# chto/linna

Hardware: AMD Instinct MI355X
Metric: emulator log-likelihood evals/sec (higher is better)
Workload: dtype f32; 1 GPU; 33-D Gaussian, 4x512 MLP emulator (33->512x4->33), nwalkers=4096 batched log-likelihood per GPU (BASELINE configs[1]); nwalkers_per_gpu=4096, launch=direct launches, parallelism=walkers sharded, 1 rank(s), no data-path collective

## Files before the change

### include/linna_hip.h

```cpp
#ifndef LINNA_HIP_H
#define LINNA_HIP_H
#include <stddef.h>
#include <stdint.h>

#ifdef __cplusplus
extern "C" {
#endif

#define LINNA_ABI_VERSION 12

typedef struct linna_ctx linna_ctx_t;
typedef struct linna_net linna_net_t;
typedef struct linna_logprob linna_logprob_t;
typedef struct linna_graph linna_graph_t;

int linna_abi_version(void);
const char* linna_last_error(void);
#define LINNA_OK 0
#define LINNA_ERR_INVALID (-1)
#define LINNA_ERR_HIP (-2)
#define LINNA_ERR_UNSUPPORTED (-3)
#define LINNA_ERR_INTERNAL (-4)
int linna_debug_raise(int kind);
int linna_ctx_create(int device, linna_ctx_t** out);
// ... 61 lines not shown
                     const float* W, int ldw, float* dX, int lddx, const float* Xmask, int ldxm,
                     float* dW, int lddw, float* db, int B, int K, int N, float scale, void* stream);

#define LINNA_LD(k) (((k) + 3) & ~3)
#define LINNA_OP_LINEAR 0
#define LINNA_OP_RESBLOCK 1
#define LINNA_OP_INSKIP 2

typedef struct {
    uint32_t struct_size;
    int op;
    int K, C, N;
    int relu;
    float alpha;
    const float *W, *b;
    const float *W1, *b1, *W2, *b2, *Ws;
    float *gW, *gb, *gW1, *gb1, *gW2, *gb2, *gWs;
} linna_layer_t;

typedef struct {
    const float* cscale; const float* cshift;
    int cexp; const float* cpost; const float* cshift2;
} linna_colmap_t;

int linna_net_create(linna_ctx_t* ctx, const linna_layer_t* layers, int nlayers, int in_size,
                     linna_net_t** out);
int linna_net_destroy(linna_net_t* net);
int linna_net_prepare(linna_net_t* net, int backward, int input_grad);
size_t linna_net_fwd_ws_bytes(const linna_net_t* net, int B);
size_t linna_net_bwd_ws_bytes(const linna_net_t* net, int B);
int linna_net_forward(linna_net_t* net, const float* X, int ldx, int B, void* ws, float* OUT, int ldo,
                      const linna_colmap_t* outmap, void* stream);
int linna_net_backward(linna_net_t* net, const float* X, int ldx, int B, void* fwd_ws, void* bwd_ws,
                       const float* dOUT, int lddo, float* dX, int lddx, int param_grads, void* stream);
int linna_net_train_launches(const linna_net_t* net, int B);
int linna_net_set_train_precision(linna_net_t* net, int precision);
int linna_net_train_precision(const linna_net_t* net, int* out);
int linna_net_stream_state(const linna_net_t* net, int* fwd, int* dx, int* dx_input);

int linna_prior_map_fwd(linna_ctx_t* ctx, const float* Z, int ldz, int B, int nin, const int* is_flat,
                        const float* a1, const float* a2, const int* log10_flag, const float* xmean,
                        const float* xstd, float* X, int ldx, float* THETA, int ldt, void* stream);
int linna_prior_map_bwd(linna_ctx_t* ctx, const float* Z, int ldz, int B, int nin, const int* is_flat,
                        const float* a1, const float* a2, const int* log10_flag, const float* xstd,
                        const float* dX, int lddx, float* dZ, int lddz, void* stream);

int linna_gauss_loglike_diag(linna_ctx_t* ctx, const float* D, int ldd, int B, int nout, const float* w,
                             const float* Z, int ldz, int nin, float temperature, float* out,
                             void* stream);
int linna_gauss_loglike_dense(linna_ctx_t* ctx, const float* D, int ldd, int B, int nout,
                              const float* S, int lds, const float* Z, int ldz, int nin,
                              float temperature, float* scratch, float* out, void* stream);

typedef struct {
    uint32_t struct_size;
    int nin, nout;
    const int* is_flat; const float* a1; const float* a2;
    const int* log10_flag; const float* xmean; const float* xstd;
    linna_colmap_t outmap;
    const float* S; int lds;
    const float* Ssym;
    const float* w;
    const float* gscale;
    float temperature;
    const float* Sfac;
} linna_logprob_desc_t;

int linna_logprob_create(linna_ctx_t* ctx, linna_net_t* net, const linna_logprob_desc_t* desc,
                         linna_logprob_t** out);
int linna_logprob_destroy(linna_logprob_t* lp);
int linna_weights_changed(linna_ctx_t* ctx);
#define LINNA_PRECISION_FP32 0
#define LINNA_PRECISION_BF16 1
int linna_logprob_set_precision(linna_logprob_t* lp, int precision);
int linna_logprob_precision(const linna_logprob_t* lp, int* out);
int linna_logprob_set_grad_precision(linna_logprob_t* lp, int precision);
int linna_logprob_grad_precision(const linna_logprob_t* lp, int* out);
int linna_logprob_set_dense_grad(linna_logprob_t* lp, int on);
int linna_logprob_dense_grad(const linna_logprob_t* lp, int* out);
int linna_engine_rows(int rows);
int linna_dense_tri(int mode);
int linna_serve_plain(int on);
int linna_serve_plain_sched(int hand);
int linna_program_plain(const linna_layer_t* layers, int nlayers, int in_size, int rows, int dense_nout);
int linna_logprob_serve_plain(linna_logprob_t* lp, int B, int* out);
int linna_logprob_grad_launches(linna_logprob_t* lp, int B, int* out);
int linna_slice_fusion(int mask);
int linna_program_describe(const linna_layer_t* layers, int nlayers, int in_size, int rows, int dense_nout, char* buf,
                           size_t n);
int linna_program_describe_grad_bf16(const linna_layer_t* layers, int nlayers, int in_size, int rows, char* buf, size_t n);
int linna_program_describe_grad_dense(const linna_layer_t* layers, int nlayers, int in_size, int nout, int tri, int rows,
                                      char* buf, size_t n);
size_t linna_logprob_ws_bytes(const linna_logprob_t* lp, int B, int with_grad);
int linna_logprob_eval(linna_logprob_t* lp, const float* Z, int ldz, int B, void* ws, float* lnP,
                       float* THETA, int ldt, void* stream);
int linna_logprob_eval_if(linna_logprob_t* lp, const float* Z, int ldz, int B, void* ws, float* lnP,
                          float* THETA, int ldt, const int* gate, void* stream);
int linna_logprob_eval_slice_points(linna_logprob_t* lp, const float* coords, int ldc, int ndim, const int* S_idx,
                                    int ns, const float* DIR, int ldd, const float* w, int nrep, float* lnP,
                                    const int* gate, void* stream);
int linna_logprob_grad(linna_logprob_t* lp, const float* Z, int ldz, int B, void* ws, float* lnP,
                       float* G, int ldg, void* stream);
int linna_logprob_grad_leapfrog(linna_logprob_t* lp, float* Q, int ldq, int B, void* ws, float* lnP, float* G, int ldg,
                                float* P, int ldp, const float* mass, float eps_kick, float eps_drift, void* stream);

typedef struct {
    uint32_t struct_size;
    int nout;
    const float* sigma; const float* ymean; const float* ystd;
    const float* data_norm;
    const float* Cinv; int ldc;
    int ylog;
} linna_loss_desc_t;

size_t linna_loss_scratch_bytes(int B, int nout);
int linna_chi2_md(linna_ctx_t* ctx, const linna_loss_desc_t* d, const float* Y, int ldy, int nrows,
                  float* scratch, float* den, void* stream);
int linna_chi2_ratio_loss_fwd_bwd(linna_ctx_t* ctx, const linna_loss_desc_t* d, const float* PRED,
                                  int ldp, const float* Y, int ldy, const float* den, const int* ROWS,
                                  int B, float* scratch, float* loss_rows, float* loss_mean,
                                  float* dPRED, int lddp, float inv_batch, void* stream);
int linna_net_prepare_loss(linna_net_t* net, const linna_loss_desc_t* d);
int linna_loss_targets(linna_ctx_t* ctx, const linna_loss_desc_t* d, const float* Y, int ldy, int nrows, float* YN, int ldyn,
                       void* stream);
int linna_net_forward_loss(linna_net_t* net, const linna_loss_desc_t* d, const float* X, int ldx, const int* ROWS, int B,
                           const int* log10_flag, const float* xmean, const float* xstd, float* XB, int ldxb, void* ws,
                           float* PRED, int ldp, const float* YN, int ldyn, const float* den, float inv_batch,
                           float* loss_rows, float* loss_mean, float* dPRED, int lddp,
                           float* hyper, int* step_dev, float beta1, float beta2, void* stream);
int linna_net_train_step(linna_net_t* net, const linna_loss_desc_t* d, const float* X, int ldx, const int* ROWS, int B,
                         const int* log10_flag, const float* xmean, const float* xstd, float* XB, int ldxb, void* fwd_ws,
                         float* PRED, int ldp, const float* YN, int ldyn, const float* den, float inv_batch,
                         float* loss_rows, float* loss_mean, float* dPRED, int lddp, void* bwd_ws,
                         float* hyper, int* step_dev, float beta1, float beta2, void* stream);
int linna_val_rows(linna_ctx_t* ctx, const linna_loss_desc_t* d, const float* PRED, int ldp,
                   const float* Y, int ldy, const float* den, int B, float* scratch, float* loss_rows,
                   float* frac_rows, void* stream);
int linna_val_metrics(linna_ctx_t* ctx, const float* loss_rows, const float* frac_rows, int n, const float* last_train_loss,
                      float* out, void* stream);
int linna_gather_xform(linna_ctx_t* ctx, const float* X, int ldx, const int* ROWS, int B, int nin,
                       const int* log10_flag, const float* xmean, const float* xstd, float* XB, int ldxb,
                       void* stream);
int linna_adamw_step(linna_ctx_t* ctx, float* p, const float* g, float* m, float* v, size_t n,
                     float* hyper, int* step_dev, float beta1, float beta2, float eps,
                     int prepared ,
                     void* stream);
int linna_net_adamw_step(linna_net_t* net, int B, float* p, const float* g, float* m, float* v, size_t n,
                         float* hyper, int* step_dev, float beta1, float beta2, float eps, int prepared, void* stream);
int linna_net_train_step_update(linna_net_t* net, const linna_loss_desc_t* d, const float* X, int ldx, const int* ROWS, int B,
                                const int* log10_flag, const float* xmean, const float* xstd, float* XB, int ldxb,
                                void* fwd_ws, float* PRED, int ldp, const float* YN, int ldyn, const float* den,
                                float inv_batch, float* loss_rows, float* loss_mean, float* dPRED, int lddp, void* bwd_ws,
                                float* params, float* m, float* v, size_t n, float* hyper, int* step_dev, float beta1,
                                float beta2, float eps, void* stream);

int linna_stretch_propose(linna_ctx_t* ctx, const float* coords, int ldc, int ndim, const int* S_idx,
                          int ns, const float* ccoords, int ldcc, const int* C_idx, int nc, uint64_t seed,
                          const int* step_dev, int stream_id, float a, float* Q, int ldq, float* factors,
                          void* stream);
int linna_stretch_accept(linna_ctx_t* ctx, float* coords, int ldc, int ndim, float* logp,
                         const int* S_idx, int ns, const float* Q, int ldq, const float* logp_new,
                         const float* factors, uint64_t seed, const int* step_dev, int stream_id,
                         int* naccept, void* stream);
int linna_stretch_half_step(linna_logprob_t* lp, float* coords, int ldc, int ndim, float* logp,
                            const int* S_idx, int ns, const float* ccoords, int ldcc, const int* C_idx,
                            int nc, uint64_t seed, const int* step_dev, int step_offset, int stream_id,
// ... 132 lines not shown
```

### linna_amd/_lib.py

```python
import ctypes as C
import os

import torch

_HERE = os.path.dirname(os.path.abspath(__file__))
LIB_PATH = os.environ.get("LINNA_LIB_PATH") or os.path.join(_HERE, "liblinna_hip.so")
ABI_VERSION = 12
RHAT_BLOCK = 128

c_float_p = C.c_void_p
c_int_p = C.c_void_p


class _Sized(C.Structure):

    def __init__(self, *a, **k):
        C.Structure.__init__(self, *a, **k)
        self.struct_size = C.sizeof(type(self))


def sized_array(cls, n):
    arr = (cls * n)()
    for i in range(n):
        arr[i].struct_size = C.sizeof(cls)
# ... 27 lines not shown
    _fields_ = [("cscale", C.c_void_p), ("cshift", C.c_void_p), ("cexp", C.c_int), ("cpost", C.c_void_p),
                ("cshift2", C.c_void_p)]


class LogprobDesc(_Sized):
    _fields_ = [("struct_size", C.c_uint32), ("nin", C.c_int), ("nout", C.c_int), ("is_flat", C.c_void_p), ("a1", C.c_void_p), ("a2", C.c_void_p),
                ("log10_flag", C.c_void_p), ("xmean", C.c_void_p), ("xstd", C.c_void_p), ("outmap", ColMap),
                ("S", C.c_void_p), ("lds", C.c_int), ("Ssym", C.c_void_p), ("w", C.c_void_p), ("gscale", C.c_void_p),
                ("temperature", C.c_float), ("Sfac", C.c_void_p)]


class HmcState(_Sized):
    _fields_ = [("struct_size", C.c_uint32), ("B", C.c_int), ("ld", C.c_int), ("seed", C.c_uint64), ("step_dev", C.c_void_p),
                ("mass", C.c_void_p), ("X", C.c_void_p), ("lnp", C.c_void_p), ("G", C.c_void_p), ("P", C.c_void_p),
                ("Q", C.c_void_p), ("lnp_new", C.c_void_p), ("Gnew", C.c_void_p), ("H0", C.c_void_p)]


class LossDesc(_Sized):
    _fields_ = [("struct_size", C.c_uint32), ("nout", C.c_int), ("sigma", C.c_void_p), ("ymean", C.c_void_p), ("ystd", C.c_void_p),
                ("data_norm", C.c_void_p), ("Cinv", C.c_void_p), ("ldc", C.c_int), ("ylog", C.c_int)]


OP_LINEAR, OP_RESBLOCK, OP_INSKIP = 0, 1, 2
COMM_ID_BYTES = 128
LAY_K, LAY_MN = 0, 1
CHEES_HEAD, CHEES_LR, CHEES_BETA1, CHEES_BETA2, CHEES_ADAM_EPS, CHEES_ALPHA_FLOOR, CHEES_MAX_STEPS = 12, 0.025, 0.9, 0.999, 1e-8, 1e-3, 64

_V, _I, _F, _SZ, _U64 = C.c_void_p, C.c_int, C.c_float, C.c_size_t, C.c_uint64
_I64, _D = C.c_int64, C.c_double
_PV = C.POINTER(C.c_void_p)

_SIGNATURES = {
    "linna_abi_version": (_I, []),
    "linna_last_error": (C.c_char_p, []),
    "linna_debug_raise": (_I, [_I]),
    "linna_ctx_create": (_I, [_I, _PV]),
    "linna_ctx_destroy": (_I, [_V]),
    "linna_stream_sync": (_I, [_V]),
    "linna_graph_begin": (_I, [_V]),
    "linna_graph_end": (_I, [_V, _PV]),
    "linna_graph_launch": (_I, [_V, _V]),
    "linna_graph_destroy": (_I, [_V]),
    "linna_event_create": (_I, [_PV]),
    "linna_event_record": (_I, [_V, _V]),
    "linna_event_elapsed_ms": (_I, [_V, _V, C.POINTER(C.c_float)]),
    "linna_event_destroy": (_I, [_V]),
    "linna_comm_unique_id": (_I, [_V]),
    "linna_comm_init": (_I, [_V, _I, _I, _V]),
    "linna_comm_destroy": (_I, [_V]),
    "linna_comm_info": (_I, [_V, C.POINTER(C.c_int), C.POINTER(C.c_int), C.POINTER(C.c_int)]),
    "linna_allreduce_sum_f32": (_I, [_V, _V, _SZ, _V]),
    "linna_allgather_f32": (_I, [_V, _V, _V, _SZ, _V]),
    "linna_broadcast_f32": (_I, [_V, _V, _SZ, _I, _V]),
    "linna_gemm_f32": (_I, [_V, C.POINTER(Gemm), _V]),
    "linna_gemm_dot_slots": (_I, [_I, _I]),
    "linna_linear_fwd": (_I, [_V, _V, _I, _V, _I, _V, _V, _I, _I, _I, _I, _I, _F, _V, _I, _V]),
    "linna_resblock_fwd": (_I, [_V, _V, _I, _V, _V, _V, _V, _V, _V, _I, _V, _I, _I, _I, _I, _I, _V]),
    "linna_linear_bwd": (_I, [_V, _V, _I, _V, _I, _V, _I, _V, _I, _V, _I, _V, _I, _V, _I, _I, _I, _F, _V]),
    "linna_net_create": (_I, [_V, C.POINTER(Layer), _I, _I, _PV]),
    "linna_net_destroy": (_I, [_V]),
    "linna_net_prepare": (_I, [_V, _I, _I]),
    "linna_net_fwd_ws_bytes": (_SZ, [_V, _I]),
    "linna_net_bwd_ws_bytes": (_SZ, [_V, _I]),
    "linna_net_forward": (_I, [_V, _V, _I, _I, _V, _V, _I, C.POINTER(ColMap), _V]),
    "linna_net_backward": (_I, [_V, _V, _I, _I, _V, _V, _V, _I, _V, _I, _I, _V]),
    "linna_net_stream_state": (_I, [_V, _V, _V, _V]),
    "linna_prior_map_fwd": (_I, [_V, _V, _I, _I, _I, _V, _V, _V, _V, _V, _V, _V, _I, _V, _I, _V]),
    "linna_prior_map_bwd": (_I, [_V, _V, _I, _I, _I, _V, _V, _V, _V, _V, _V, _I, _V, _I, _V]),
    "linna_gauss_loglike_diag": (_I, [_V, _V, _I, _I, _I, _V, _V, _I, _I, _F, _V, _V]),
    "linna_gauss_loglike_dense": (_I, [_V, _V, _I, _I, _I, _V, _I, _V, _I, _I, _F, _V, _V, _V]),
    "linna_logprob_create": (_I, [_V, _V, C.POINTER(LogprobDesc), _PV]),
    "linna_logprob_destroy": (_I, [_V]),
    "linna_weights_changed": (_I, [_V]),
    "linna_logprob_set_precision": (_I, [_V, _I]),
    "linna_logprob_precision": (_I, [_V, _V]),
    "linna_logprob_set_grad_precision": (_I, [_V, _I]),
    "linna_logprob_grad_precision": (_I, [_V, _V]),
    "linna_logprob_set_dense_grad": (_I, [_V, _I]),
    "linna_logprob_dense_grad": (_I, [_V, _V]),
    "linna_engine_rows": (_I, [_I]),
    "linna_dense_tri": (_I, [_I]),
    "linna_serve_plain": (_I, [_I]),
    "linna_serve_plain_sched": (_I, [_I]),
    "linna_program_plain": (_I, [_V, _I, _I, _I, _I]),
    "linna_logprob_serve_plain": (_I, [_V, _I, _V]),
    "linna_logprob_grad_launches": (_I, [_V, _I, _V]),
    "linna_slice_fusion": (_I, [_I]),
    "linna_net_train_launches": (_I, [_V, _I]),
    "linna_net_set_train_precision": (_I, [_V, _I]),
    "linna_net_train_precision": (_I, [_V, _V]),
    "linna_program_describe": (_I, [_V, _I, _I, _I, _I, _V, C.c_size_t]),
    "linna_program_describe_grad_bf16": (_I, [_V, _I, _I, _I, _V, C.c_size_t]),
    "linna_program_describe_grad_dense": (_I, [_V, _I, _I, _I, _I, _I, _V, C.c_size_t]),
    "linna_logprob_ws_bytes": (_SZ, [_V, _I, _I]),
    "linna_logprob_eval": (_I, [_V, _V, _I, _I, _V, _V, _V, _I, _V]),
    "linna_logprob_grad": (_I, [_V, _V, _I, _I, _V, _V, _V, _I, _V]),
    "linna_logprob_grad_leapfrog": (_I, [_V, _V, _I, _I, _V, _V, _V, _I, _V, _I, _V, _F, _F, _V]),
    "linna_loss_scratch_bytes": (_SZ, [_I, _I]),
    "linna_chi2_md": (_I, [_V, C.POINTER(LossDesc), _V, _I, _I, _V, _V, _V]),
    "linna_chi2_ratio_loss_fwd_bwd": (_I, [_V, C.POINTER(LossDesc), _V, _I, _V, _I, _V, _V, _I, _V, _V, _V, _V, _I, _F, _V]),
    "linna_net_prepare_loss": (_I, [_V, C.POINTER(LossDesc)]),
    "linna_loss_targets": (_I, [_V, C.POINTER(LossDesc), _V, _I, _I, _V, _I, _V]),
    "linna_net_forward_loss": (_I, [_V, C.POINTER(LossDesc), _V, _I, _V, _I, _V, _V, _V, _V, _I, _V, _V, _I, _V, _I, _V, _F, _V, _V, _V, _I,
                                    _V, _V, _F, _F, _V]),
    "linna_net_train_step": (_I, [_V, C.POINTER(LossDesc), _V, _I, _V, _I, _V, _V, _V, _V, _I, _V, _V, _I, _V, _I, _V, _F, _V, _V, _V, _I,
                                  _V, _V, _V, _F, _F, _V]),
    "linna_net_train_step_update": (_I, [_V, C.POINTER(LossDesc), _V, _I, _V, _I, _V, _V, _V, _V, _I, _V, _V, _I, _V, _I, _V, _F, _V, _V, _V, _I,
                                         _V, _V, _V, _V, _SZ, _V, _V, _F, _F, _F, _V]),
    "linna_val_rows": (_I, [_V, C.POINTER(LossDesc), _V, _I, _V, _I, _V, _I, _V, _V, _V, _V]),
    "linna_val_metrics": (_I, [_V, _V, _V, _I, _V, _V, _V]),
    "linna_gather_xform": (_I, [_V, _V, _I, _V, _I, _I, _V, _V, _V, _V, _I, _V]),
    "linna_adamw_step": (_I, [_V, _V, _V, _V, _V, _SZ, _V, _V, _F, _F, _F, _I, _V]),
    "linna_net_adamw_step": (_I, [_V, _I, _V, _V, _V, _V, _SZ, _V, _V, _F, _F, _F, _I, _V]),
    "linna_stretch_propose": (_I, [_V, _V, _I, _I, _V, _I, _V, _I, _V, _I, _U64, _V, _I, _F, _V, _I, _V, _V]),
    "linna_stretch_accept": (_I, [_V, _V, _I, _I, _V, _V, _I, _V, _I, _V, _V, _U64, _V, _I, _V, _V]),
    "linna_logprob_eval_if": (_I, [_V, _V, _I, _I, _V, _V, _V, _I, _V, _V]),
    "linna_logprob_eval_slice_points": (_I, [_V, _V, _I, _I, _V, _I, _V, _I, _V, _I, _V, _V, _V]),
    "linna_stretch_half_step": (_I, [_V, _V, _I, _I, _V, _V, _I, _V, _I, _V, _I, _U64, _V, _I, _I, _F, _V, _V]),
    "linna_stretch_run": (_I, [_V, _V, _I, _I, _V, _I, _V, _I, _I, _U64, _V, _I, _F, _V, _V, _V, _V]),
    "linna_chain_append_t": (_I, [_V, _V, _I, _I, _I, _I, _I, _V, _I, _I64, _V]),
    "linna_acorr_update": (_I, [_V, _V, _I, _I, _I, _I64, _I64, _I64, _I64, _I, _I, _V, _V, _I, _V]),
    "linna_acorr_scratch_bytes": (_SZ, [_I, _I, _I]),
    "linna_acorr_tau": (_I, [_V, _V, _I, _I, _I, _I, _I64, _I64, _I, _V, _V, _D, _V, _V, _V]),
    "linna_chain_meanstd": (_I, [_V, _V, _I, _I, _I, _I64, _I64, _I64, _V, _V]),
    "linna_chain_block_moments": (_I, [_V, _V, _I, _I, _I64, _I64, _V, _V]),
    "linna_chain_rhat": (_I, [_V, _V, _I, _I, _I, _I64, _I64, _V, _I64, _V, _V]),
    "linna_acorr_ess_scratch_bytes": (_SZ, [_I, _I, _I]),
    "linna_acorr_ess": (_I, [_V, _V, _I, _I, _I, _I, _I64, _I64, _I, _V, _V, _V, _V, _V]),
    "linna_chain_rank_rhat_scratch_bytes": (_SZ, [_I, _I, _I64, _I]),
    "linna_chain_rank_rhat": (_I, [_V, _V, _I, _I, _I, _I64, _I64, _V, _SZ, _V, _V, _V]),
    "linna_hmc_init": (_I, [_V, _I, _I, _V, _U64, _V, _V, _V, _I, _V, _I, _V, _V]),
    "linna_hmc_start": (_I, [_V, _I, _I, _V, _U64, _V, _V, _V, _I, _V, _I, _F, _F, _V, _I, _V, _I, _V, _I, _V, _V]),
    "linna_hmc_kick_drift": (_I, [_V, _I, _I, _V, _F, _F, _V, _I, _V, _I, _V, _I, _V]),
    "linna_hmc_accept": (_I, [_V, _I, _I, _V, _U64, _V, _V, _V, _I, _V, _I, _V, _V, _I, _V, _V, _I, _V, _V, _V, _V]),
    "linna_hmc_start_eps": (_I, [_V, _I, _I, _V, _U64, _V, _I, _V, _V, _I, _V, _I, _V, _F, _F, _V, _I, _V, _I, _V, _I, _V, _V]),
    "linna_hmc_kick_drift_eps": (_I, [_V, _I, _I, _V, _V, _F, _F, _V, _I, _V, _I, _V, _I, _V]),
    "linna_logprob_grad_leapfrog_eps": (_I, [_V, _V, _I, _I, _V, _V, _V, _I, _V, _I, _V, _V, _F, _F, _V]),
    "linna_hmc_accept_adapt": (_I, [_V, _I, _I, _V, _U64, _V, _I, _V, _V, _I, _V, _I, _V, _V, _I, _V, _V, _I, _V, _V, _V, _V,
                                    _V, _V, _V, _V, _V, _I, _F, _V, _V, _V]),
    "linna_hmc_run": (_I, [_V, _V, _V, _V, _V, _V, _V, _V, _I, _F, _I, _I, _I, _V, _V, _V, _V, _V]),
    "linna_hmc_find_epsilon": (_I, [_V, _V, _V, _V, _V, _V, _V, _I, _I, _V]),
    "linna_hmc_moments": (_I, [_V, _I, _I, _V, _I, _V, _V]),
    "linna_hmc_mass_from_moments": (_I, [_V, _I, _V, _V, _I, _V]),
    "linna_hmc_run_moments": (_I, [_V, _V, _V, _V, _V, _V, _V, _V, _I, _F, _I, _I, _I, _V, _V, _V, _V, _V, _V]),
    "linna_hmc_comoments_doubles": (_SZ, [_I]),
    "linna_hmc_comoments": (_I, [_V, _I, _I, _V, _I, _V, _V]),
    "linna_hmc_chol_from_comoments": (_I, [_V, _I, _V, _V, _I, _V, _I, _V]),
    "linna_hmc_kick_drift_dense": (_I, [_V, _I, _I, _V, _I, _V, _F, _F, _V, _I, _V, _I, _V, _I, _V, _I, _V]),
    "linna_hmc_run_dense": (_I, [_V, _V, _V, _V, _I, _V, _V, _V, _V, _V, _I, _F, _I, _I, _I, _V, _V, _V, _V, _V, _V]),
    "linna_hmc_find_epsilon_dense": (_I, [_V, _V, _V, _V, _I, _V, _V, _V, _V, _I, _I, _V]),
    "linna_hmc_chees_doubles": (_SZ, [_I]),
    "linna_hmc_chees_begin": (_I, [_V, _I, _I, _V, _I, _V, _V, _V]),
    "linna_hmc_chees_end": (_I, [_V, _I, _I, _V, _V, _I, _V, _I, _V, _I, _V, _V, _V, _V, _I, _D, _I, _V]),
    "linna_step_increment": (_I, [_V, _V, _V]),
    "linna_slice_init": (_I, [_V, _V, _V, _I, _V, _I, _V, _I, _I, _V, _U64, _V, _I, _V, _I, _V, _V, _V, _V, _I, _V]),
    "linna_slice_points": (_I, [_V, _V, _I, _I, _V, _I, _V, _I, _V, _V, _I, _I, _V]),
    "linna_slice_expand": (_I, [_V, _V, _V, _V, _V, _V, _V, _I, _V, _I, _V]),
    "linna_slice_draw": (_I, [_V, _V, _V, _V, _V, _V, _I, _U64, _V, _I, _I, _I, _V]),
    "linna_slice_shrink": (_I, [_V, _V, _V, _V, _V, _V, _V, _V, _V, _I, _V, _I, _I, _V]),
    "linna_slice_commit": (_I, [_V, _V, _I, _I, _V, _V, _I, _V, _I, _V, _V, _V]),
    "linna_slice_half_step": (_I, [_V, _V, _I, _I, _V, _V, _I, _V, _I, _V, _I, _V, _U64, _V, _I, _V, _I, _V, _I, _V, _I, _V, _V, _V, _V, _V, _V, _V, _I, _I, _V, _I, _V]),
}
EXPORTED = tuple(_SIGNATURES)

_lib = None

# ... 65 lines not shown
        raise LinnaHipError("expected dtype %s, got %s" % (dtype, t.dtype))
    if not t.is_contiguous():
        raise LinnaHipError("expected a contiguous tensor")
    return C.c_void_p(t.data_ptr())


def iptr(t):
    return ptr(t, torch.int32)


def ld4(w):
    return (int(w) + 3) & ~3


class _Stage(object):
    __slots__ = ("name", "t0")

    def __init__(self, name):
        self.name = name

    def __enter__(self):
        if stage_profile.current is not None:
            import time
            self.t0 = time.perf_counter()
        return self

    def __exit__(self, *exc):
        d = stage_profile.current
        if d is not None:
            import time
            d[self.name] = d.get(self.name, 0.0) + time.perf_counter() - self.t0
        return False


def stage(name):
    return _Stage(name)


class stage_profile(object):
    current = None

    def __init__(self, d):
        self.d = d

    def __enter__(self):
        self.prev, stage_profile.current = stage_profile.current, self.d
        return self.d

    def __exit__(self, *exc):
        stage_profile.current = self.prev
        return False


class quiet_gc(object):

    def __enter__(self):
        import gc
        self.on = gc.isenabled() and os.environ.get("LINNA_QUIET_GC", "1") != "0"
        if self.on:
            gc.freeze()
        return self

    def __exit__(self, *exc):
        import gc
        if self.on:
            gc.unfreeze()
        return False


def slice_fusion(mask=-1):
    prev = load().linna_slice_fusion(int(mask))
    if prev < 0:
        check(prev)
    return prev


def serve_plain_sched(hand=-1):
    prev = load().linna_serve_plain_sched(int(hand))
    if prev < 0:
        check(prev)
    return prev


def serve_plain(on=-1):
    prev = load().linna_serve_plain(int(on))
    if prev < 0:
        check(prev)
    return prev


def engine_rows(rows=0):
    prev = load().linna_engine_rows(int(rows))
    if prev < 0:
        check(prev)
    return prev
```

### linna_amd/csrc/api.hip

```cpp
#include "common.h"

#include <stdarg.h>
#include <stdio.h>
#include <string.h>
#include <cstring>
#include <string>
#include <vector>
#include <atomic>
#include <new>
#include <stdlib.h>

namespace linna {

static thread_local std::string g_err;

void set_error(const char* fmt, ...) {
    char buf[512];
    va_list ap;
    va_start(ap, fmt);
    vsnprintf(buf, sizeof buf, fmt, ap);
    va_end(ap);
    g_err = buf;
}

// ... 1053 lines not shown
    if (lp->d.outmap.cexp) { set_error("logprob_set_grad_precision: no bf16 gradient: the ypositive (exp) output map has no gradient path"); return LINNA_ERR_UNSUPPORTED; }
    if (!lp->d.w || !lp->d.gscale) { set_error("logprob_set_grad_precision: no bf16 gradient: it needs a diagonal likelihood with gscale"); return LINNA_ERR_UNSUPPORTED; }
    const NsPlan g = net_stream_plan(NS_GRAD_INPUT_BF16, n->Lfull.data(), (int)n->Lfull.size(), n->in_size);
    if (!g.ok) {
        set_error("logprob_set_grad_precision: no bf16 gradient for this network: %s", g.why ? g.why : "not eligible");
        return LINNA_ERR_UNSUPPORTED;
    }
    if (!lp->packed_gbf.ready() && lp->packed_gbf.alloc(g.packed_floats) != LINNA_OK) {
        set_error("logprob_set_grad_precision: hipMalloc(bf16 gradient weight stream) failed");
        return LINNA_ERR_HIP;
    }
    lp->grad_precision = precision;
    return LINNA_OK;
} LINNA_CATCH_INT
int linna_logprob_grad_precision(const linna_logprob_t* lp, int* out) try {
    if (!lp || !out) { set_error("logprob_grad_precision: null argument"); return LINNA_ERR_INVALID; }
    *out = lp->grad_precision;
    return LINNA_OK;
} LINNA_CATCH_INT
int linna_logprob_set_dense_grad(linna_logprob_t* lp, int on) try {
    if (!lp) { set_error("logprob_set_dense_grad: null handle"); return LINNA_ERR_INVALID; }
    if (on != 0 && on != 1) { set_error("logprob_set_dense_grad: %d (0 layered, 1 one launch)", on); return LINNA_ERR_INVALID; }
    if (!on) { lp->dense_grad = false; return LINNA_OK; }
    const linna_net* n = lp->net;
    const linna_logprob_desc_t& d = lp->d;
    if (lp->bf16()) { set_error("logprob_set_dense_grad: a bf16 handle has no dense-covariance gradient (fp32 only)"); return LINNA_ERR_UNSUPPORTED; }
    if (d.w) { set_error("logprob_set_dense_grad: the covariance is diagonal: its gradient is one launch already where the network has the program"); return LINNA_ERR_UNSUPPORTED; }
    if (d.outmap.cexp) { set_error("logprob_set_dense_grad: the ypositive (exp) output map has no gradient path"); return LINNA_ERR_UNSUPPORTED; }
    if (!d.Sfac) {
        set_error("logprob_set_dense_grad: no factored inverse covariance (Sfac): it is not positive definite, or LINNA_DENSE_FACTORED=0");
        return LINNA_ERR_UNSUPPORTED;
    }
    if (n->has_inskip) { set_error("logprob_set_dense_grad: an input-skip network has no one-launch gradient"); return LINNA_ERR_UNSUPPORTED; }
    const NsDense dn = lp->dense();
    const NsPlan g = net_stream_plan(NS_GRAD_INPUT_DENSE, n->L.data(), (int)n->L.size(), n->in_size, &dn);
    if (!g.ok) {
        set_error("logprob_set_dense_grad: no one-launch dense gradient for this network: %s", g.why ? g.why : "not eligible");
        return LINNA_ERR_UNSUPPORTED;
    }
    if (!lp->packed_gd.ready() && lp->packed_gd.alloc(g.packed_floats) != LINNA_OK) {
        set_error("logprob_set_dense_grad: hipMalloc(dense gradient weight stream) failed");
        return LINNA_ERR_HIP;
    }
    for (int e = 0; e < 3; ++e) lp->gd_fits[e] = net_stream_grad_dense_fits(n->L.data(), (int)n->L.size(), n->in_size, &dn, 16 >> e);
    lp->dense_grad = true;
    return LINNA_OK;
} LINNA_CATCH_INT
int linna_logprob_dense_grad(const linna_logprob_t* lp, int* out) try {
    if (!lp || !out) { set_error("logprob_dense_grad: null argument"); return LINNA_ERR_INVALID; }
    *out = lp->dense_grad ? 1 : 0;
    return LINNA_OK;
} LINNA_CATCH_INT
int linna_program_describe_grad_dense(const linna_layer_t* layers, int nlayers, int in_size, int nout, int tri, int rows, char* buf, size_t n) try {
    if (!layers || nlayers < 1 || !buf || !n || nout < 1 || tri < 0 || tri > 2) { set_error("program_describe_grad_dense: bad arguments"); return LINNA_ERR_INVALID; }
    TRY(check_layers(layers, nlayers, "program_describe_grad_dense"));
    if (layers[nlayers - 1].N != nout) { set_error("program_describe_grad_dense: %d columns for a network of %d outputs", nout, layers[nlayers - 1].N); return LINNA_ERR_INVALID; }
    static float dummy[2];
    const NsDense dn{dummy, (nout + 3) & ~3, dummy + 1, dummy + 1, 1, tri};
    return net_stream_describe(NS_GRAD_INPUT_DENSE, layers, nlayers, in_size, &dn, rows, buf, n);
} LINNA_CATCH_INT
int linna_program_describe_grad_bf16(const linna_layer_t* layers, int nlayers, int in_size, int rows, char* buf, size_t n) try {
    if (!layers || nlayers < 1 || !buf || !n) { set_error("program_describe_grad_bf16: bad arguments"); return LINNA_ERR_INVALID; }
    TRY(check_layers(layers, nlayers, "program_describe_grad_bf16"));
    return net_stream_describe(NS_GRAD_INPUT_BF16, layers, nlayers, in_size, nullptr, rows, buf, n);
} LINNA_CATCH_INT
int linna_program_describe(const linna_layer_t* layers, int nlayers, int in_size, int rows, int dense_nout, char* buf, size_t n) try {
    if (!layers || nlayers < 1 || !buf || !n) { set_error("program_describe: bad arguments"); return LINNA_ERR_INVALID; }
    TRY(check_layers(layers, nlayers, "program_describe"));
    static float dummy;
    if (dense_nout == -1) return net_stream_describe(ns_grad_kind(layers, nlayers), layers, nlayers, in_size, nullptr, rows, buf, n);
    const int dn_cols = dense_nout < -1 ? -dense_nout : dense_nout;
    NsDense dn{&dummy, (dn_cols + 3) & ~3, nullptr, nullptr, dense_nout < -1 ? 1 : 0, net_stream_dense_tri(-1)};
    if (dn_cols > 0) return net_stream_describe(NS_SERVE_DENSE, layers, nlayers, in_size, &dn, rows, buf, n);
    return net_stream_describe(NS_SERVE, layers, nlayers, in_size, nullptr, rows, buf, n);
} LINNA_CATCH_INT
int linna_serve_plain(int on) try {
    if (on < -1 || on > 1) { set_error("linna_serve_plain: %d (-1 query, 0 or 1)", on); return LINNA_ERR_INVALID; }
    return net_stream_serve_plain(on);
} LINNA_CATCH_INT
int linna_serve_plain_sched(int hand) try {
    if (hand < -1 || hand > 1) { set_error("linna_serve_plain_sched: %d (-1 query, 0 or 1)", hand); return LINNA_ERR_INVALID; }
    return net_stream_serve_plain_sched(hand);
} LINNA_CATCH_INT
int linna_program_plain(const linna_layer_t* layers, int nlayers, int in_size, int rows, int dense_nout) try {
    if (!layers || nlayers < 1) { set_error("program_plain: bad arguments"); return LINNA_ERR_INVALID; }
    TRY(check_layers(layers, nlayers, "program_plain"));
    if (dense_nout != 0) return 0;
    return net_stream_program_plain(NS_SERVE, layers, nlayers, in_size, nullptr, rows) ? 1 : 0;
} LINNA_CATCH_INT
int linna_logprob_serve_plain(linna_logprob_t* lp, int B, int* out) try {
    if (!lp || !out || B < 1) { set_error("logprob_serve_plain: bad arguments"); return LINNA_ERR_INVALID; }
    static float lnP;
    *out = lp_eval_route(lp, false).route == LP_EVAL_ONE &&
           net_stream_takes_plain(lp->kind(), net_layers(lp->net, lp->kind()), lp_output(lp), NsRun{nullptr, 0, B, &lnP}, nullptr, nullptr,
                                  net_stream_rows(B), nullptr);
    return LINNA_OK;
} LINNA_CATCH_INT
int linna_dense_tri(int mode) try {
    if (mode < -1 || mode > 2) { set_error("linna_dense_tri: %d (-1 query, 0, 1 or 2)", mode); return LINNA_ERR_INVALID; }
    return net_stream_dense_tri(mode);
} LINNA_CATCH_INT
static std::atomic<int> g_slice_fusion{7};
static bool slice_derive_enabled() { return (g_slice_fusion.load() & 1) != 0; }
int linna_slice_fusion(int mode) try {
    if (mode < -1 || mode > 7) { set_error("linna_slice_fusion: %d (-1 query, or a mask of bits 0-2)", mode); return LINNA_ERR_INVALID; }
    return mode < 0 ? g_slice_fusion.load() : g_slice_fusion.exchange(mode);
} LINNA_CATCH_INT
int linna_engine_rows(int rows) try {
    const int prev = net_stream_force_rows(rows);
    if (prev < 0) { set_error("linna_engine_rows: %d (0, 4, 8 or 16)", rows); return LINNA_ERR_INVALID; }
    if (prev != rows) g_weights_epoch.fetch_add(1);
    return prev;
} LINNA_CATCH_INT
size_t linna_logprob_ws_bytes(const linna_logprob_t* lp, int B, int with_grad) try {
    return (lp_layout(lp, B, with_grad).total + 16) * sizeof(float);
} LINNA_CATCH_SIZE

int linna_logprob_eval(linna_logprob_t* lp, const float* Z, int ldz, int B, void* ws, float* lnP, float* TH, int ldt,
                       void* stream) try {
    if (!lp || !Z || !ws || !lnP || B < 1) { set_error("logprob_eval: bad arguments"); return LINNA_ERR_INVALID; }
    return lp_forward(lp, NsRun{Z, ldz, B, lnP, nullptr, TH, ldt}, static_cast<float*>(ws), lp_layout(lp, B, 0), stream, false);
} LINNA_CATCH_INT

int linna_logprob_eval_if(linna_logprob_t* lp, const float* Z, int ldz, int B, void* ws, float* lnP, float* TH, int ldt,
                          const int* gate, void* stream) try {
    if (!lp || !Z || !ws || !lnP || B < 1) { set_error("logprob_eval_if: bad arguments"); return LINNA_ERR_INVALID; }
    return lp_forward(lp, NsRun{Z, ldz, B, lnP, gate, TH, ldt}, static_cast<float*>(ws), lp_layout(lp, B, 0), stream, false);
} LINNA_CATCH_INT

struct SliceDerive { const float* Z0; const float* L; const float* R; const float* Ze; int m, nt; uint64_t seed; const int* step_dev; int stream_id; const int* flags; };
struct SlicePoints { const float* coords; int ldc, ndim; const int* S_idx; int ns; const float* DIR; int ldd; };
static int lp_eval_slice_points(linna_logprob_t* lp, const SlicePoints& pt, const float* w, int nrep, float* lnP, const int* gate,
                                const int* list, const int* count, int mul, int b_engine, void* stream, const SliceDerive* sd = nullptr,
                                const SliceBegin* sb = nullptr) {
    if (!lp || !pt.coords || !pt.S_idx || !pt.DIR || !w || !lnP || pt.ns < 1 || nrep < 1) {
        set_error("logprob_eval_slice_points: bad arguments"); return LINNA_ERR_INVALID;
    }
    if (pt.ndim != lp->d.nin) { set_error("logprob_eval_slice_points: ndim %d, log-probability has %d parameters", pt.ndim, lp->d.nin); return LINNA_ERR_INVALID; }
    if (!lp_runs_fused_move(lp)) {
        set_error("logprob_eval_slice_points: this log-probability does not run the whole-network kernel");
        return LINNA_ERR_UNSUPPORTED;
    }
    const float* packed = nullptr; int rows = 16;
    TRY(lp_refresh_stream(lp, b_engine > 0 ? b_engine : nrep * pt.ns, stream, &packed, &rows));
    NsMove mv{const_cast<float*>(pt.coords), pt.ldc, nullptr, pt.S_idx, w, 0, list, pt.ns, 0ull, count, mul, 0, 0.f, nullptr, 1};
    mv.sb = sb;
    if (sd) {
        mv.sl_Z0 = sd->Z0; mv.sl_L = sd->L; mv.sl_R = sd->R; mv.sl_Zt = sd->Ze; mv.sl_m = sd->m; mv.sl_nt = sd->nt;
        mv.sl_seed = sd->seed; mv.sl_step = sd->step_dev; mv.sl_stream = sd->stream_id; mv.sl_flags = sd->flags;
    }
    return lp_launch(lp, packed, rows, NsRun{pt.DIR, pt.ldd, nrep * pt.ns, lnP, gate}, &mv, nullptr, stream);
}
int linna_logprob_eval_slice_points(linna_logprob_t* lp, const float* coords, int ldc, int ndim, const int* S_idx, int ns,
                                    const float* DIR, int ldd, const float* w, int nrep, float* lnP, const int* gate,
                                    void* stream) try {
    return lp_eval_slice_points(lp, SlicePoints{coords, ldc, ndim, S_idx, ns, DIR, ldd}, w, nrep, lnP, gate, nullptr, nullptr, 0, 0, stream);
} LINNA_CATCH_INT

int linna_slice_half_step(linna_logprob_t* lp, float* coords, int ldc, int ndim, float* logp, const int* S_idx, int ns,
                          const float* ccoords, int ldcc, const int* C_idx, int nc, const float* mu, uint64_t seed,
                          int* step_dev, int half, const int* m_sched, int nexp_rounds, const int* nt_sched, int nshr_rounds,
                          float* DIR, int ldd, float* state, int* flags, float* W, float* Wd, float* Zt, int* list, int* counters,
                          int zero_totals, int bump_step, const int* expect_rows, int maxsteps, void* stream) try {
    if (!lp || !coords || !logp || !S_idx || !ccoords || !C_idx || !mu || !step_dev || !DIR || !state || !flags || !W || !Wd ||
        !Zt || !list || !counters || ns < 1 || nc < 2 || !m_sched || !nt_sched || nexp_rounds < 1 || nshr_rounds < 1 || (half != 0 && half != 1)) {
        set_error("slice_half_step: bad arguments"); return LINNA_ERR_INVALID;
// ... 697 lines not shown
```

### linna_amd/csrc/common.h

```cpp
#pragma once
#include <hip/hip_runtime.h>
#include <stdint.h>
#include <exception>
#include "../../include/linna_hip.h"


typedef float f32x4 __attribute__((ext_vector_type(4)));
typedef float f32x16 __attribute__((ext_vector_type(16)));

namespace linna {

struct U4 { uint32_t x, y, z, w; };
__device__ __forceinline__ U4 philox4x32_10(U4 c, uint32_t k0, uint32_t k1) {
#pragma unroll
    for (int r = 0; r < 10; ++r) {
        const uint64_t p0 = (uint64_t)0xD2511F53u * c.x;
        const uint64_t p1 = (uint64_t)0xCD9E8D57u * c.z;
        U4 n;
        n.x = (uint32_t)(p1 >> 32) ^ c.y ^ k0;
        n.y = (uint32_t)p1;
        n.z = (uint32_t)(p0 >> 32) ^ c.w ^ k1;
        n.w = (uint32_t)p0;
        c = n;
        k0 += 0x9E3779B9u; k1 += 0xBB67AE85u;
// ... 212 lines not shown
                        const float* xstd, float* XB, int ldxb, hipStream_t s);
int launch_colsum(const float* dZ, int ld, int B, int N, float scale, float* db, hipStream_t s);
int launch_adamw(float* p, const float* g, float* m, float* v, size_t n, float* hyper, int* step_dev, float b1, float b2,
                 float eps, hipStream_t s);
int launch_adamw_prepare(float* hyper, int* step_dev, float b1, float b2, hipStream_t s);
int launch_stretch_propose(const float* coords, int ldc, int ndim, const int* S, int ns, const float* ccoords, int ldcc,
                           const int* C, int nc, uint64_t seed, const int* step_dev, int stream_id, float a, float* Q,
                           int ldq, float* factors, hipStream_t s);
int launch_stretch_accept(float* coords, int ldc, int ndim, float* logp, const int* S, int ns, const float* Q, int ldq,
                          const float* lp_new, const float* factors, uint64_t seed, const int* step_dev, int stream_id,
                          int* naccept, hipStream_t s);
int launch_hmc_start(int B, int ndim, const float* mass, uint64_t seed, const int* step_dev, const float* lnp, const float* P0,
                     int ldp0, const float* G, int ldg, float ek, float ed, const float* X, int ldx, float* P, int ldp, float* Q,
                     int ldq, float* H0, hipStream_t s, const float* eps = nullptr, int step_off = 0);
int launch_hmc_kick_drift(int B, int ndim, const float* mass, float ek, float ed, const float* G, int ldg, float* P,
                          int ldp, float* Q, int ldq, hipStream_t s, const float* eps = nullptr);
struct HmcAdapt { float* eps; float* epsbar; float* Hbar; const float* mu; int* m; int Madapt; float delta; };
int launch_hmc_accept(int B, int ndim, const float* mass, uint64_t seed, const int* step_dev, int step_off, const float* H0,
                      const float* P, int ldp, const float* Qn, int ldq, const float* lnp_new, const float* Gn, int ldg,
                      const float* U, float* X, int ldx, float* lnp, float* G, int* naccept, float* alpha,
                      const HmcAdapt& ad, float* chain, float* logps, hipStream_t s);
int launch_hmc_find_eps_init(int B, int ndim, uint64_t seed, const int* step_dev, int step_off, float* R0, int ldr, float* eps,
                             int* state, hipStream_t s);
int launch_hmc_find_eps(int B, int ndim, const float* mass, const float* H0, const float* P, int ldp, const float* lnp_new,
                        const float* Gn, int ldg, float* eps, int* state, int* nactive, hipStream_t s);
int launch_hmc_moments(int B, int ndim, const float* X, int ldx, double* mom, hipStream_t s);
int launch_hmc_mass_from_moments(int ndim, double* mom, float* mass, int reset, hipStream_t s);
int launch_hmc_comoments(int B, int ndim, const float* X, int ldx, double* mom, hipStream_t s);
int launch_hmc_chol_from_comoments(int ndim, double* mom, float* Cm, int ldc, int* info, int reset, hipStream_t s);
int launch_hmc_kick_drift_dense(int B, int ndim, const float* Cm, int ldc, const float* eps, float ek, float ed, const float* G,
                                int ldg, float* W, int ldw, const float* X, int ldx, float* Q, int ldq, hipStream_t s);
int launch_hmc_chees_begin(int B, int ndim, const float* X, int ldx, double* state, double* r0, hipStream_t s);
int launch_hmc_chees_end(int B, int ndim, const float* mass, const float* Cm, int ldc, const float* Q, int ldq, const float* P, int ldp,
                         const float* alpha, const double* r0, double* state, float* eps, int M, double delta, int max_steps,
                         hipStream_t s);
int launch_slice_points(const float* coords, int ldc, int ndim, const int* S, int ns, const float* DIR, int ldd,
                        const float* w, float* Q, int ldq, int nrep, hipStream_t s);
int launch_slice_expand(const float* Z0, const float* ZL, const float* ZR, float* L, float* R, int* flags, int ns,
                        int* counters, int slot, hipStream_t s);
int launch_slice_draw(const float* L, const float* R, const int* S, float* W, const int* flags, int ns, uint64_t seed,
                      const int* step_dev, int stream_id, int round, int ntrial, hipStream_t s);
int launch_slice_shrink(const float* Z0, const float* Zt, float* L, float* R, const float* W, int* flags, float* Wacc,
                        float* Zacc, int ns, int* counters, int slot, int ntrial, hipStream_t s);
int launch_slice_begin(const SliceBegin& b, const int* S, int ns, int ndim, float* W, hipStream_t s);
int launch_slice_expand_multi(const float* Z0, const float* Zt, float* L, float* R, const int* S, int* flags, int ns, int m,
                              int m_next, int* counters, int slot, int prev_slot, float* W, float* Wd, int* list, uint64_t seed,
                              const int* step_dev, int stream_id_shrink, int ntrial, hipStream_t s);
int launch_slice_shrink_multi(const SliceRound& a, hipStream_t s);
int launch_slice_commit(float* coords, int ldc, int ndim, float* logp, const int* S, int ns, const float* DIR, int ldd,
                        const float* Wacc, const float* Zacc, hipStream_t s);
int launch_step_increment(int* step, hipStream_t s);

struct NsDense { const float* S; int lds; const float* cscale; const float* cshift; int factored = 0;
                 int tri = 2; };
int net_stream_dense_tri(int mode);
enum NsKind {
    NS_SERVE,
    NS_SERVE_DENSE,
    NS_SERVE_BF16,
    NS_STORE,
    NS_TRAIN_FWD,
    NS_DX,
    NS_DX_INPUT,
    NS_GRAD_INPUT,
    NS_TRAIN_STEP,
    NS_TRAIN_STEP_BF16,
    NS_GRAD_INPUT_BF16,
    NS_GRAD_INPUT_WIDE,
    NS_GRAD_INPUT_DENSE,
};
inline bool ns_kind_full_layers(NsKind k) { return k == NS_SERVE || k == NS_SERVE_DENSE || k == NS_SERVE_BF16; }
struct NsPlan { bool ok; size_t packed_floats; bool grad_ok; const char* why; };
NsPlan net_stream_plan(NsKind kind, const linna_layer_t* layers, int nl, int in_size, const NsDense* dn = nullptr);
int net_stream_rows(int B);
int net_stream_force_rows(int rows);
inline NsKind ns_grad_kind(const linna_layer_t* layers, int nl) { return nl >= 1 && layers[nl - 1].N > 64 ? NS_GRAD_INPUT_WIDE : NS_GRAD_INPUT; }
bool net_stream_grad_fits(const linna_layer_t* layers, int nl, int in_size, int rows);
bool net_stream_grad_dense_fits(const linna_layer_t* layers, int nl, int in_size, const NsDense* dn, int rows);
int launch_net_stream_pack(NsKind kind, const linna_layer_t* layers, int nl, int in_size, float* packed, int rows, const NsDense* dn,
                           hipStream_t s);
int net_stream_describe(NsKind kind, const linna_layer_t* layers, int nl, int in_size, const NsDense* dn, int rows, char* buf, size_t n);
int net_stream_serve_plain(int on);
int net_stream_serve_plain_sched(int hand);
bool net_stream_program_plain(NsKind kind, const linna_layer_t* layers, int nl, int in_size, const NsDense* dn, int rows);
bool net_stream_launch_plain_ok(bool cscale, bool cshift, bool w, bool cexp, bool lnP, bool D, bool TH, bool gate);
struct NsNet { const linna_layer_t* layers; int nl, in_size; };
struct NsInput { int nin; const int* is_flat; const float* a1; const float* a2; const int* lg; const float* xmean; const float* xstd; };
struct NsOutput { const float* cscale; const float* cshift; const float* cpost; const float* cshift2; const float* w; float T; };
struct NsRun { const float* Z; int ldz; int B; float* lnP; const int* gate = nullptr; float* TH = nullptr; int ldt = 0; float* D = nullptr; int ldd = 0; };
struct NsOpBufs { float* y; int ldy; float* t; int ldt; const float* x; int ldx; const float* gate; float* dprev; int ldp; float* dt; int lddt; };
struct NsPost { const float* rows; int n; float scale; float* out; int* step; float* hyper; float b1, b2; };
int launch_net_stream_dx(const NsNet& net, const float* packed, const float* dOUT, int lddo, int B, const NsOpBufs* ops, int with_input,
                         int rows, hipStream_t s, const NsPost* post = nullptr);
struct NsMove {
    float* coords; int ldc; float* logp; const int* S;
    const float* cc; int ldcc; const int* C; int nc;
    unsigned long long seed; const int* step; int step_off; int stream; float a; int* naccept;
    int slice;
    float* chain = nullptr; float* lps = nullptr;
    const float* sl_Z0 = nullptr; const float* sl_L = nullptr; const float* sl_R = nullptr; const float* sl_Zt = nullptr;
    int sl_m = 0, sl_nt = 0; unsigned long long sl_seed = 0; const int* sl_step = nullptr; int sl_stream = 0;
    const int* sl_flags = nullptr;
    const SliceBegin* sb = nullptr;
};
int launch_net_stream_store(const NsNet& net, const float* packed, const float* X, int ldx, int B, const NsOpBufs* ops,
                            const float* cscale, const float* cshift, int rows, hipStream_t s);
struct NsTrainLoss { const float* YN; int ldyn;
                     const float* den; float inv_batch; float* loss_rows; float* dP; int lddp; };
struct NsBatch { const float* X; int ldx; const int* ROWS; int B; const int* lg; const float* xmean; const float* xstd; float* XB; int ldxb; };
int launch_loss_targets(const float* Y, int ldy, int n, const linna_loss_desc_t& d, float* YN, int ldyn, hipStream_t s);
int launch_net_stream_train(const NsNet& net, const float* packed, const NsBatch& b, const NsOpBufs* ops, const NsTrainLoss& L,
                            const NsDense& dn, int rows, hipStream_t s);
int launch_net_stream_train_bwd(const NsNet& net, const float* packed, const NsBatch& b, const NsOpBufs* ops, const NsTrainLoss& L,
                                const NsDense& dn, int rows, hipStream_t s, const NsPost* post,
                                bool bf = false);
struct NsLeap { float* P; int ldp; float* Q; const float* mass; float ek, ed; const float* eps; };
struct NsGrad { const float* gscale; float* G; int ldg; NsLeap leap; };
constexpr int AS_MAXR = 26, AS_MAXW = 14, AS_MAXB = 12;
struct AsPlace { float* out; float scale; int trans, koff, ncols, type, ncg, steps, G, first0, first1; };
struct AsMat { int N, ld; AsPlace pl[2]; };
struct AsBias { float* out; float scale; int N; };
struct AsRange { unsigned off4, n4, blk0; short kind, idx; };
struct AsArgs { AsRange r[AS_MAXR]; AsMat w[AS_MAXW]; AsBias b[AS_MAXB]; int nr, small; unsigned nblocks; };
__device__ __forceinline__ size_t as_slot(const AsPlace& q, int small, int nn, int kk) {
    const int nl = nn & 63, ks = kk >> 4, kr = kk & 15;
    int w, g;
    if (q.type == 0) { w = (nn & 511) >> 6; g = ((nn >> 9) ? q.first1 : q.first0) + ks; }
    else { const int kp = ks / q.steps; w = kp * q.ncg + (nn >> 6); g = q.first0 + (ks - kp * q.steps); }
    const int t = small ? kr >> 2 : nl >> 4, lane = small ? nl : (nl & 15) + 16 * (kr >> 2);
    return ((((size_t)w * q.G + g) * 4 + t) * 64 + lane) * 4 + (kr & 3);
}
__device__ __forceinline__ size_t as_slot_bf16(const AsPlace& q, int nn, int kk) {
    const int nl = nn & 63, ks = kk >> 5, kr = kk & 31;
    int w, g;
    if (q.type == 0) { w = (nn & 511) >> 6; g = ((nn >> 9) ? q.first1 : q.first0) + ks; }
    else { const int kp = ks / q.steps; w = kp * q.ncg + (nn >> 6); g = q.first0 + (ks - kp * q.steps); }
    return ((((size_t)w * q.G + g) * 4 + (kr >> 3)) * 64 + nl) * 8 + (kr & 7);
}
typedef __bf16 bf16x4_t __attribute__((ext_vector_type(4)));
__device__ __forceinline__ void adamw_one(float& pi, float gi, float& mi, float& vi, float lr, float wd, float bc1, float sbc2,
                                          float beta1, float beta2, float eps) {
    pi = pi * (1.f - lr * wd);
    mi = mi + (gi - mi) * (1.f - beta1);
    vi = vi * beta2 + (1.f - beta2) * gi * gi;
    const float denom = sqrtf(vi) / sbc2 + eps;
    pi = pi - (lr / bc1) * (mi / denom);
}
int net_stream_adamw_args(const linna_layer_t* layers, int nl, int in_size, int rows, const float* params, size_t nflat,
                          float* s_fwd, const NsDense* dn, float* s_dx, AsArgs* out, int merged = 0);
int launch_adamw_streams(const AsArgs& a, float* p, const float* g, float* m, float* v, const float* hyper, float b1, float b2,
                         float eps, hipStream_t s, bool bf = false);
int launch_net_stream_grad2(const NsNet& net, const float* packed, const NsRun& r, const NsInput& in, const NsOutput& out, const NsGrad& gr,
                            int rows, hipStream_t s, bool bf = false);
int launch_net_stream_grad_dense(const NsNet& net, const float* packed, const NsRun& r, const NsInput& in, float T, const NsGrad& gr,
                                 int rows, const NsDense& dn, hipStream_t s);
bool net_stream_takes_plain(NsKind kind, const NsNet& net, const NsOutput& out, const NsRun& r, const NsMove* mv, const NsGrad* gr, int rows,
                            const NsDense* dn);
int launch_net_stream(NsKind kind, const NsNet& net, const float* packed, const NsRun& r, const NsInput& in, const NsOutput& out,
                      const NsMove* mv, const NsGrad* gr, int rows, const NsDense* dn, hipStream_t s);

int launch_chain_append_t(const float* block, int ldb, int nsteps, int nw, int ndim, int wstride, float* CT, int nwp,
                          int64_t row0, hipStream_t s);
int launch_acorr_update(const float* CT, int nd, int nwp, int nwc, int64_t a0, int64_t a1, int64_t lo, int64_t hi, int k0, int k1,
                        double* S, double* T, int remove, hipStream_t s);
size_t acorr_scratch_doubles(int nser, int kuse, int nd);
int launch_acorr_tau(const float* CT, int ndim, int nwp, int nwc, int nlive, int64_t lo, int64_t hi, int kuse, const double* S,
// ... 33 lines not shown
```

### linna_amd/csrc/net_program.h

```cpp
#pragma once
#include "common.h"
#include <memory>
#include <vector>

namespace linna {

constexpr int NS_ROWS = 16;
constexpr int NS_NW = 8;
constexpr int NS_NT = 4;
constexpr int NS_MAXSEG = 20;
constexpr int NS_SEGCAP = 22;
constexpr int NS_MAXRUN = 40;
constexpr unsigned NS_STEP_B = NS_NT * 1024;
constexpr int NS_LDS_BYTES = 160 * 1024;
constexpr int AS_BLOCK = 64;
enum { NS_WIDE = 0, NS_SPLIT = 1, NS_SIDE = 2 };

struct NsSeg {
    int type, steps, passes, bias_off;
    int dst_col, relu, kslice, zext;
    int ncg_log2;
    int mask_store, mask_apply;
    int x0_n;
    int x0_col;
    int kcl, side_off;
};

struct NsPackSeg {
    const float* Wa; int lda, Ka, Kapad;
    const float* Wb; int ldb, Kb; float alpha;
    const float* b; float bscale;
    const float* b2; float b2scale;
    int N, type, steps, passes, bias_off, bias_pad, ncg;
    int transA;
    int transB;
    const float* rscale; const float* rshift;
    int kc, side_off;
    int koff2;
    const float* kscale;
};

struct NsProgram {
    std::vector<NsPackSeg> pack;
    std::vector<NsSeg> seg;
    int G = 0, LD = 0, kpad0 = 0, nout = 0, bias_total = 0;
    int Gstride = 0, nseg_f = 0, mask_slots = 0;
    size_t packed_floats = 0;
    int dense = 0, u_col = 0, u_same = 0;
    int x0_keep = 0;
    size_t side_f4 = 0;
    bool bf = false;
    int f32seg = -1;
    bool ok = false, grad_ok = false;
    bool dxi_ok = false;
    bool train_ok = false;
    int nops = 0;
    std::vector<int> seg_op, seg_hidden;
    size_t lds_for(int rows, bool grad) const;
};

int ns_seg_steps(const NsSeg& s);
int ns_forced_rows_resolved();
typedef std::shared_ptr<const NsProgram> NsProgramRef;
NsProgramRef ns_program(NsKind kind, const linna_layer_t* layers, int nl, int in_size, const NsDense* dn, int rows);

bool ns_program_plain(const NsProgram& p);
int ns_seg_cols(const NsProgram& p, const linna_layer_t* layers, int i);
struct NsGates {
    int gbit[NS_SEGCAP], mbit[NS_SEGCAP];
    int ncols = 0;
    bool ok = true;
    size_t lds0 = 0, lds = 0;
};
NsGates ns_gates(const NsProgram& p, const linna_layer_t* layers, int nl, int rows);
}
```

### linna_amd/csrc/net_program.hip

```cpp
#include "net_program.h"
#include <stdlib.h>
#include <algorithm>
#include <atomic>
#include <cstring>
#include <mutex>
#include <string>
#include <unordered_map>

namespace linna {

size_t NsProgram::lds_for(int rows, bool grad) const {
    size_t b = (size_t)(2 * rows * LD + ((bias_total + 3) & ~3)) * sizeof(float) + 128 + (x0_keep ? 4096 : 0);
#ifdef NS_STAMPS
    b += NS_NW * 32 * 8;
#endif
    return b + (grad ? (size_t)mask_slots * 64 * NS_NW * sizeof(unsigned) : 0);
}

static int ceil16(int k) { return (k + 15) & ~15; }
int ns_seg_steps(const NsSeg& s) {
    if (s.type == NS_WIDE && s.zext < 0) return 2 * s.steps - 60;
    return s.type == NS_WIDE && s.zext > 0 ? s.steps + (s.passes - 1) * s.zext : s.steps * s.passes;
}
static int ns_switch(std::atomic<int>& sw, const char* name, int dflt, bool (*valid)(int)) {
// ... 331 lines not shown
    p.ok = ns_sizes(p, maxext);
    return p;
}

static std::atomic<int> g_forced_rows{-1};
int ns_forced_rows_resolved() { return ns_switch(g_forced_rows, "LINNA_NS_ROWS", 0, [](int v) { return v == 4 || v == 8 || v == 16; }); }
int net_stream_force_rows(int rows) {
    if (rows != 0 && rows != 4 && rows != 8 && rows != 16) return -1;
    (void)ns_forced_rows_resolved();
    return g_forced_rows.exchange(rows);
}

static bool ns_side(NsKind kind, int rows) {
    return rows == 16 && (kind == NS_SERVE || kind == NS_SERVE_DENSE || kind == NS_GRAD_INPUT || kind == NS_GRAD_INPUT_WIDE || kind == NS_GRAD_INPUT_DENSE);
}

static NsProgram ns_build_kind(NsKind kind, const linna_layer_t* layers, int nl, int in_size, const NsDense* dn, bool side) {
    NsBuildOpts o;
    o.side = side;
    switch (kind) {
    case NS_SERVE: case NS_STORE: o.bwd = NS_BWD_MLP; break;
    case NS_SERVE_DENSE: case NS_TRAIN_FWD: o.dense = true; break;
    case NS_SERVE_BF16: o.bf = true; if (dn) return NsProgram(); break;
    case NS_DX: o.forward = false; break;
    case NS_DX_INPUT: o.forward = false; o.dx_first = 0; break;
    case NS_GRAD_INPUT: o.bwd = NS_BWD_INPUT; break;
    case NS_GRAD_INPUT_WIDE: o.bwd = NS_BWD_INPUT; o.wide_out = true; break;
    case NS_GRAD_INPUT_DENSE: o.bwd = NS_BWD_INPUT; o.dense = true; break;
    case NS_GRAD_INPUT_BF16: o.bwd = NS_BWD_INPUT; o.bf = true; if (dn) return NsProgram(); break;
    case NS_TRAIN_STEP: case NS_TRAIN_STEP_BF16: o.dense = true; o.bwd = NS_BWD_TRAIN; o.bf = kind == NS_TRAIN_STEP_BF16; break;
    }
    NsProgram p = ns_build_one(layers, nl, in_size, o, dn);
    if (!p.ok && o.bwd == NS_BWD_MLP) {
        o.bwd = NS_BWD_NONE;
        p = ns_build_one(layers, nl, in_size, o, dn);
    }
    if (side && !(p.ok && ((kind != NS_GRAD_INPUT && kind != NS_GRAD_INPUT_WIDE && kind != NS_GRAD_INPUT_DENSE) || p.dxi_ok))) return ns_build_kind(kind, layers, nl, in_size, dn, false);
    return p;
}
NsProgramRef ns_program(NsKind kind, const linna_layer_t* layers, int nl, int in_size, const NsDense* dn, int rows) {
    static std::mutex mu;
    static std::unordered_map<std::string, NsProgramRef> cache;
    const bool side = ns_side(kind, rows);
    std::string key;
    key.reserve((size_t)nl * sizeof(linna_layer_t) + 64);
    key.append(reinterpret_cast<const char*>(layers), (size_t)nl * sizeof(linna_layer_t));
    const int hdr[4] = {nl, in_size, (int)kind, side ? 1 : 0};
    key.append(reinterpret_cast<const char*>(hdr), sizeof(hdr));
    if (dn) {
        const void* const ptrs[3] = {dn->S, dn->cscale, dn->cshift};
        key.append(reinterpret_cast<const char*>(ptrs), sizeof(ptrs));
        key.append(reinterpret_cast<const char*>(&dn->lds), sizeof(int));
        key.append(reinterpret_cast<const char*>(&dn->factored), sizeof(int));
        key.append(reinterpret_cast<const char*>(&dn->tri), sizeof(int));
    }
    std::lock_guard<std::mutex> lock(mu);
    auto it = cache.find(key);
    if (it != cache.end()) return it->second;
    if (cache.size() >= 256) cache.clear();
    NsProgramRef p = std::make_shared<const NsProgram>(ns_build_kind(kind, layers, nl, in_size, dn, side));
    cache.emplace(std::move(key), p);
    return p;
}

bool ns_program_plain(const NsProgram& p) {
    if (!p.ok || p.bf || p.dense || p.x0_keep || p.side_f4 || p.nseg_f < 1) return false;
    for (int i = 0; i < p.nseg_f; ++i) {
        const NsSeg& g = p.seg[i];
        if (g.type != NS_WIDE && g.type != NS_SPLIT) return false;
        if (g.x0_col || (g.type == NS_WIDE && (g.zext || g.kslice))) return false;
    }
    return true;
}
bool net_stream_program_plain(NsKind kind, const linna_layer_t* layers, int nl, int in_size, const NsDense* dn, int rows) {
    return kind == NS_SERVE && rows == 16 && ns_program_plain(*ns_program(kind, layers, nl, in_size, dn, rows));
}
bool net_stream_launch_plain_ok(bool cscale, bool cshift, bool w, bool cexp, bool lnP, bool D, bool TH, bool gate) {
    return cscale && cshift && w && !cexp && lnP && !D && !TH && !gate;
}
static std::atomic<int> g_serve_plain{1};
int net_stream_serve_plain(int on) { return on < 0 ? g_serve_plain.load() : g_serve_plain.exchange(on ? 1 : 0); }
static std::atomic<int> g_serve_plain_sched{1};
int net_stream_serve_plain_sched(int hand) { return hand < 0 ? g_serve_plain_sched.load() : g_serve_plain_sched.exchange(hand ? 1 : 0); }

int ns_seg_cols(const NsProgram& p, const linna_layer_t* layers, int i) {
    if (p.seg_op[i] >= p.nops) return p.nout;
    const linna_layer_t& l = layers[p.seg_op[i]];
    return p.seg_hidden[i] ? l.C : i < p.nseg_f ? l.N : l.K;
}
NsGates ns_gates(const NsProgram& p, const linna_layer_t* layers, int nl, int rows) {
    NsGates g;
    for (int i = 0; i < NS_SEGCAP; ++i) g.gbit[i] = g.mbit[i] = -1;
    for (int i = 0; i < p.nseg_f; ++i) {
        const int op = p.seg_op[i];
        if (op >= nl || (!p.seg_hidden[i] && op == nl - 1)) continue;
        g.gbit[i] = g.ncols;
        g.ncols += (ns_seg_cols(p, layers, i) + 63) & ~63;
    }
    for (int i = p.nseg_f; i < (int)p.seg.size(); ++i) {
        const int op = p.seg_op[i];
        const bool hidden = p.seg_hidden[i] != 0;
        if (op >= nl) continue;
        if (!hidden && !(op > 0 && (layers[op - 1].op == LINNA_OP_RESBLOCK || layers[op - 1].relu))) continue;
        const int src = hidden ? op : op - 1;
        for (int j = 0; j < p.nseg_f; ++j)
            if (p.seg_op[j] == src && (p.seg_hidden[j] != 0) == hidden) g.mbit[i] = g.gbit[j];
        if (g.mbit[i] < 0) g.ok = false;
    }
    g.lds0 = (p.lds_for(rows, true) + 7) & ~(size_t)7;
    g.lds = g.lds0 + (size_t)rows * (g.ncols / 32) * sizeof(unsigned);
    return g;
}

static size_t ns_grad_lds(const linna_layer_t* layers, int nl, int in_size, int rows) {
    const NsProgramRef pref = ns_program(ns_grad_kind(layers, nl), layers, nl, in_size, nullptr, rows);
    return pref->ok && pref->dxi_ok ? ns_gates(*pref, layers, nl, rows).lds : 0;
}
bool net_stream_grad_fits(const linna_layer_t* layers, int nl, int in_size, int rows) {
    const size_t lds = ns_grad_lds(layers, nl, in_size, rows);
    return lds && lds <= (size_t)NS_LDS_BYTES;
}

static size_t ns_grad_dense_lds(const linna_layer_t* layers, int nl, int in_size, const NsDense* dn, int rows) {
    const NsProgramRef pref = ns_program(NS_GRAD_INPUT_DENSE, layers, nl, in_size, dn, rows);
    if (!pref->ok || !pref->dxi_ok) return 0;
    const NsGates g = ns_gates(*pref, layers, nl, rows);
    return g.ok ? g.lds : 0;
}
bool net_stream_grad_dense_fits(const linna_layer_t* layers, int nl, int in_size, const NsDense* dn, int rows) {
    const size_t lds = ns_grad_dense_lds(layers, nl, in_size, dn, rows);
    return lds && lds <= (size_t)NS_LDS_BYTES;
}

static const char* ns_bf16_refusal(const NsProgram& p, const linna_layer_t* layers, int nl, int in_size) {
    int width = 0;
    for (int i = 0; i < nl; ++i) width = std::max(width, std::max(layers[i].N, layers[i].op == LINNA_OP_RESBLOCK ? layers[i].C : 0));
    if (in_size > 256) return "more than 256 network inputs: outside the whole-network kernel";
    if (width > 1024) return "a layer wider than 1024: outside the whole-network kernel";
    if (nl < 1 || layers[0].op != LINNA_OP_LINEAR) return "the first op is not a linear layer (the bf16 input split needs one)";
    if (!p.ok) return "the network does not fit the bf16 program of the whole-network kernel";
    return nullptr;
}
NsPlan net_stream_plan(NsKind kind, const linna_layer_t* layers, int nl, int in_size, const NsDense* dn) {
    const NsProgramRef pref = ns_program(kind, layers, nl, in_size, dn, 0);
    const NsProgram& p = *pref;
    NsPlan r{p.ok, p.packed_floats, p.grad_ok, nullptr};
    if (kind == NS_TRAIN_STEP) r.ok = p.ok && p.train_ok;
    if (kind == NS_TRAIN_STEP_BF16) {
        r.why = ns_bf16_refusal(p, layers, nl, in_size);
        if (!r.why && !p.train_ok) r.why = "the network has no merged training step (one layer only)";
        r.ok = r.why == nullptr;
    }
    if (kind == NS_GRAD_INPUT || kind == NS_GRAD_INPUT_WIDE) {
        r.ok = p.ok && p.dxi_ok && ns_gates(p, layers, nl, NS_ROWS).lds <= (size_t)NS_LDS_BYTES;
        for (int rows = 8; kind == NS_GRAD_INPUT_WIDE && rows >= 4; rows >>= 1) r.ok = r.ok || net_stream_grad_fits(layers, nl, in_size, rows);
        r.packed_floats = std::max(r.packed_floats, ns_program(kind, layers, nl, in_size, dn, 16)->packed_floats);
    }
    if (kind == NS_GRAD_INPUT_DENSE) {
        bool inskip = false;
        for (int i = 0; i < nl; ++i) inskip = inskip || layers[i].op == LINNA_OP_INSKIP;
        bool fits = false;
        for (int rows = 16; rows >= 4; rows >>= 1) fits = fits || net_stream_grad_dense_fits(layers, nl, in_size, dn, rows);
        if (inskip) r.why = "an input-skip network has no one-launch gradient";
        else if (in_size > 64) r.why = "more than 64 network inputs: outside the one-launch gradient";
        else if (!dn || !dn->S || !dn->factored) r.why = "the dense one-launch gradient needs the factored inverse covariance";
        else if (!fits) r.why = "the program of the dense one-launch gradient fits no engine (segments, LDS or widths)";
// ... 167 lines not shown
```

### linna_amd/csrc/net_stream.hip

```cpp
#include "net_program.h"
#include <stdlib.h>
#include <type_traits>
#include <cstring>
#include <algorithm>

namespace linna {

typedef __bf16 bf16x8 __attribute__((ext_vector_type(8)));
typedef short s16x4 __attribute__((ext_vector_type(4)));

#ifndef NS_R
#define NS_R 6
#endif
#ifndef NS_PRE
#define NS_PRE 2
#endif
struct NsArgs {
    const float* Z; int ldz; int B; int nin;
    const int* is_flat; const float* a1; const float* a2; const int* lg;
    const float* xmean; const float* xstd;
    const float* packed;
    int G, nseg, LD, kpad0, nout, bias_total;
    int Gstride, nseg_f;
    const float* gscale; float* Gout; int ldg;
// ... 117 lines not shown
    const int c = (int)j - S.bias_off;
    float bv = (c < S.N && S.b) ? S.bscale * S.b[c] : 0.f;
    if (c < S.N && S.b2) bv += S.b2scale * S.b2[c];
    if (c < S.N && S.rscale) bv *= S.rscale[c];
    if (c < S.N && S.rshift) bv += S.rshift[c];
    p.out[nw4 * 4 + j] = bv;
}

__global__ void ns_pack_side_kernel(NsPackArgs p) {
    const size_t idx = (size_t)blockIdx.x * blockDim.x + threadIdx.x;
    size_t base = 0;
    for (int si = 0; si < p.nseg; ++si) {
        const NsPackSeg& S = p.seg[si];
        if (S.type != NS_SIDE) continue;
        const size_t n4 = (size_t)NS_NW * S.steps * NS_NT * 64;
        if (idx >= base + n4) { base += n4; continue; }
        size_t q = idx - base;
        const int lane = (int)(q & 63); q >>= 6;
        const int t = (int)(q % NS_NT); q /= NS_NT;
        const int st = (int)(q % S.steps);
        const int w = (int)(q / S.steps);
        const int tpc = NS_NT / S.kc;
        const int n = 16 * (t % tpc) + (lane & 15);
        const int k0 = 16 * (S.kc * (w * S.steps + st) + t / tpc) + 4 * (lane >> 4);
        f32x4 v = {0.f, 0.f, 0.f, 0.f};
        if (n < S.N) {
#pragma unroll
            for (int e = 0; e < 4; ++e) {
                const int k = k0 + e;
                if (S.Wa) { if (k < S.Ka) v[e] = S.Wa[(size_t)n * S.lda + k]; }
                else if (k < S.Kb) v[e] = S.alpha * (S.transB ? S.Wb[(size_t)k * S.ldb + n] : S.Wb[(size_t)n * S.ldb + k]);
            }
        }
        reinterpret_cast<f32x4*>(p.out + S.side_off)[idx - base] = v;
        return;
    }
}

__device__ __forceinline__ float ns_prior_theta(float z, int flat, float a1, float a2) {
    float u = 0.5f * (1.f + erff(z / 1.41421356237309515f));
    asm volatile("" : "+v"(u));
    return (flat ? u : z) * a2 + a1;
}

template <int R, int MOVE, bool GRAD, int STORE, int ROWS, bool BF = false>
__global__ __launch_bounds__(64 * NS_NW, 1) void net_stream_kernel(NsArgs a) {
    constexpr bool EPS = false, PLAIN = false, WOUT = false, DGR = false;
#include "net_stream_body.inc"
}
template <int R, int MOVE, bool GRAD, int STORE, int ROWS, bool BF>
__global__ __launch_bounds__(64 * NS_NW, 1) void net_stream_eps_kernel(NsArgs a) {
    static_assert(!BF && GRAD && (STORE == 0 || STORE == 2) && MOVE == 0, "the fp32 one-launch gradients only");
    constexpr bool EPS = true, PLAIN = false, WOUT = false, DGR = false;
#include "net_stream_body.inc"
}
template <int R, int MOVE, bool GRAD, int STORE, int ROWS, bool BF, bool EPSV>
__global__ __launch_bounds__(64 * NS_NW, 1) void net_stream_wide_kernel(NsArgs a) {
    static_assert(!BF && GRAD && STORE == 2 && MOVE == 0, "the fp32 one-launch gradient of any network only");
    constexpr bool EPS = EPSV, PLAIN = false, WOUT = true, DGR = false;
#include "net_stream_body.inc"
}
template <int R, int MOVE, bool GRAD, int STORE, int ROWS, bool BF, bool EPSV>
__global__ __launch_bounds__(64 * NS_NW, 1) void net_stream_dense_kernel(NsArgs a) {
    static_assert(!BF && GRAD && STORE == 2 && MOVE == 0, "the fp32 one-launch gradient of any network only");
    constexpr bool EPS = EPSV, PLAIN = false, WOUT = false, DGR = true;
#include "net_stream_body.inc"
}
template <int R>
__global__ __launch_bounds__(64 * NS_NW, 1) void net_stream_plain_kernel(NsArgs a) {
    constexpr int MOVE = 0, STORE = 0, ROWS = 16;
    constexpr bool GRAD = false, BF = false, EPS = false, PLAIN = true, WOUT = false, DGR = false;
#include "net_stream_body.inc"
}
#if NS_R == 6
#define NS_HAVE_PLACED 1
template <int R>
__global__ __launch_bounds__(64 * NS_NW, 1) void net_stream_placed_kernel(NsArgs a) {
    constexpr int MOVE = 0, STORE = 0, ROWS = 16;
    constexpr bool GRAD = false, BF = false, EPS = false, PLAIN = true, WOUT = false, DGR = false;
#define NS_BODY_HAND
#include "net_stream_body.inc"
#undef NS_BODY_HAND
}
#endif
template <int R, int MOVE, bool GRAD, int STORE, int ROWS, bool BF>
__global__ __launch_bounds__(64 * NS_NW, 1) void net_stream_train_bf16_kernel(NsArgs a) {
    static_assert(BF && GRAD && STORE == 3 && ROWS == 4 && MOVE == 0, "the bf16 training step only");
    constexpr bool EPS = false, PLAIN = false, WOUT = false, DGR = false;
#include "net_stream_body.inc"
}
template <int R, int MOVE, bool GRAD, int STORE, int ROWS, bool BF>
__global__ __launch_bounds__(64 * NS_NW, 1) void net_stream_slice_bf16_kernel(NsArgs a) {
    static_assert(BF && !GRAD && STORE == 0 && MOVE == 2, "the bf16 slice evaluation only");
    constexpr bool EPS = false, PLAIN = false, WOUT = false, DGR = false;
#define NS_BODY_SLICE_BF16
#include "net_stream_body.inc"
#undef NS_BODY_SLICE_BF16
}
template <int R, int MOVE, bool GRAD, int STORE, int ROWS, bool BF>
__global__ __launch_bounds__(64 * NS_NW, 1) void net_stream_grad_bf16_kernel(NsArgs a) {
    static_assert(BF && GRAD && STORE == 2 && MOVE == 0, "the bf16 one-launch gradient only");
    constexpr bool EPS = false, PLAIN = false, WOUT = false, DGR = false;
#define NS_BODY_GRAD_BF16
#include "net_stream_body.inc"
#undef NS_BODY_GRAD_BF16
}
template <int R, int MOVE, bool GRAD, int STORE, int ROWS, bool BF>
__global__ __launch_bounds__(64 * NS_NW, 1) void net_stream_eps_bf16_kernel(NsArgs a) {
    static_assert(BF && GRAD && STORE == 2 && MOVE == 0, "the bf16 one-launch gradient only");
    constexpr bool EPS = true, PLAIN = false, WOUT = false, DGR = false;
#define NS_BODY_GRAD_BF16
#include "net_stream_body.inc"
#undef NS_BODY_GRAD_BF16
}

int net_stream_rows(int B) {
    const int forced = ns_forced_rows_resolved();
    if (forced) return forced;
    static int ncu = 0;
    if (!ncu) {
        int dev = 0; hipDeviceProp_t pr;
        ncu = (hipGetDevice(&dev) == hipSuccess && hipGetDeviceProperties(&pr, dev) == hipSuccess && pr.multiProcessorCount > 0)
                  ? pr.multiProcessorCount : 256;
    }
    return B <= 4 * ncu ? 4 : B <= 8 * ncu ? 8 : 16;
}

int launch_net_stream_pack(NsKind kind, const linna_layer_t* layers, int nl, int in_size, float* packed, int rows, const NsDense* dn,
                           hipStream_t s) {
    const NsProgramRef pref = ns_program(kind, layers, nl, in_size, dn, rows);
    const NsProgram& p = *pref;
    if (!p.ok) { set_error("net_stream: network not eligible"); return LINNA_ERR_UNSUPPORTED; }
    NsPackArgs a;
    ::memset(static_cast<void*>(&a), 0, sizeof(a));
    a.nseg = (int)p.seg.size(); a.G = p.Gstride; a.bias_total = p.bias_total; a.out = packed;
    a.small = rows < 16;
    a.bf = p.bf ? 1 : 0; a.f32seg = p.f32seg;
    int nrun = 0, first = 0;
    for (int i = 0; i < a.nseg; ++i) {
        a.seg[i] = p.pack[i];
        if (p.seg[i].type == NS_SIDE) continue;
        if (p.seg[i].type == NS_WIDE && p.seg[i].zext < 0) {
            a.run_seg[nrun] = i; a.run_pass[nrun] = 0; a.run_first[nrun] = first;
            first += ns_seg_steps(p.seg[i]); ++nrun;
            continue;
        }
        for (int ps = 0; ps < p.seg[i].passes; ++ps) {
            a.run_seg[nrun] = i; a.run_pass[nrun] = ps; a.run_first[nrun] = first;
            first += (ps > 0 && p.seg[i].type == NS_WIDE && p.seg[i].zext > 0) ? p.seg[i].zext : p.seg[i].steps; ++nrun;
        }
    }
    a.run_first[nrun] = first; a.nrun = nrun;
    const size_t total = (size_t)NS_NW * p.Gstride * NS_NT * 64 + (size_t)p.bias_total;
    hipLaunchKernelGGL(ns_pack_kernel, dim3((unsigned)((total + 255) / 256)), dim3(256), 0, s, a);
    if (p.side_f4) hipLaunchKernelGGL(ns_pack_side_kernel, dim3((unsigned)((p.side_f4 + 255) / 256)), dim3(256), 0, s, a);
    return check_hip(hipGetLastError(), "net_stream pack launch");
}

typedef void (*NsKernel)(NsArgs);
enum NsVariant { NV_SERVE, NV_STRETCH, NV_SLICE, NV_GRAD_MLP, NV_GRAD2, NV_STORE, NV_DX, NV_TRAIN_FWD, NV_TRAIN_STEP };
enum : unsigned { NF_BF16 = 1, NF_EPS = 2, NF_WIDE = 4, NF_PLAIN = 8, NF_PLACED = 16, NF_DENSE = 32 };
struct NsEntry { NsVariant v; unsigned flags; NsKernel k[3]; const char* what; const char* stamps_lacks; bool attr_set[3]; };
#define NS_ENGINES(K, MOVE, GRAD, STORE, ...) \
    {K<NS_R, MOVE, GRAD, STORE, 16, __VA_ARGS__>, K<NS_R, MOVE, GRAD, STORE, 8, __VA_ARGS__>, K<NS_R, MOVE, GRAD, STORE, 4, __VA_ARGS__>}
static NsEntry ns_table[] = {
    {NV_SERVE, 0, NS_ENGINES(net_stream_kernel, 0, false, 0, false), "net_stream launch"},
    {NV_SERVE, NF_BF16, NS_ENGINES(net_stream_kernel, 0, false, 0, true), "net_stream launch"},
    {NV_SERVE, NF_PLAIN, {net_stream_plain_kernel<NS_R>, nullptr, nullptr}, "net_stream plain launch"},
#ifdef NS_HAVE_PLACED
    {NV_SERVE, NF_PLAIN | NF_PLACED, {net_stream_placed_kernel<NS_R>, nullptr, nullptr}, "net_stream plain launch (hand-placed step)"},
#endif
    {NV_STRETCH, 0, NS_ENGINES(net_stream_kernel, 1, false, 0, false), "net_stream launch"},
    {NV_STRETCH, NF_BF16, NS_ENGINES(net_stream_kernel, 1, false, 0, true), "net_stream launch"},
    {NV_SLICE, 0, NS_ENGINES(net_stream_kernel, 2, false, 0, false), "net_stream launch"},
    {NV_SLICE, NF_BF16, NS_ENGINES(net_stream_slice_bf16_kernel, 2, false, 0, true), "net_stream bf16 slice launch", "bf16 slice evaluation"},
    {NV_GRAD_MLP, 0, NS_ENGINES(net_stream_kernel, 0, true, 0, false), "net_stream launch"},
    {NV_GRAD_MLP, NF_EPS, NS_ENGINES(net_stream_eps_kernel, 0, true, 0, false), "net_stream launch"},
    {NV_GRAD2, 0, NS_ENGINES(net_stream_kernel, 0, true, 2, false), "net_stream launch"},
    {NV_GRAD2, NF_EPS, NS_ENGINES(net_stream_eps_kernel, 0, true, 2, false), "net_stream launch"},
    {NV_GRAD2, NF_WIDE, NS_ENGINES(net_stream_wide_kernel, 0, true, 2, false, false), "net_stream wide-output gradient launch"},
    {NV_GRAD2, NF_WIDE | NF_EPS, NS_ENGINES(net_stream_wide_kernel, 0, true, 2, false, true), "net_stream wide-output gradient launch"},
    {NV_GRAD2, NF_DENSE, NS_ENGINES(net_stream_dense_kernel, 0, true, 2, false, false), "net_stream dense-covariance gradient launch"},
    {NV_GRAD2, NF_DENSE | NF_EPS, NS_ENGINES(net_stream_dense_kernel, 0, true, 2, false, true), "net_stream dense-covariance gradient launch"},
    {NV_GRAD2, NF_BF16, NS_ENGINES(net_stream_grad_bf16_kernel, 0, true, 2, true), "net_stream bf16 gradient launch", "bf16 gradient"},
    {NV_GRAD2, NF_BF16 | NF_EPS, NS_ENGINES(net_stream_eps_bf16_kernel, 0, true, 2, true), "net_stream bf16 gradient launch", "bf16 gradient"},
    {NV_STORE, 0, NS_ENGINES(net_stream_kernel, 0, false, 1, false), "net_stream launch"},
    {NV_DX, 0, NS_ENGINES(net_stream_kernel, 0, false, 2, false), "net_stream launch"},
    {NV_TRAIN_FWD, 0, NS_ENGINES(net_stream_kernel, 0, false, 3, false), "net_stream launch"},
    {NV_TRAIN_STEP, 0, {nullptr, nullptr, net_stream_kernel<NS_R, 0, true, 3, 4, false>}, "net_stream launch"},
    {NV_TRAIN_STEP, NF_BF16, {nullptr, nullptr, net_stream_train_bf16_kernel<NS_R, 0, true, 3, 4, true>}, "net_stream bf16 training launch", "bf16 training step"},
};
#undef NS_ENGINES
static int ns_kernel(NsVariant v, unsigned flags, int rows, NsEntry** entry, int* slot) {
    for (NsEntry& e : ns_table) {
        if (e.v != v || e.flags != flags) continue;
#ifdef NS_STAMPS
        if (e.stamps_lacks) { set_error("net_stream: the NS_STAMPS build has no %s", e.stamps_lacks); return LINNA_ERR_UNSUPPORTED; }
#endif
        const int i = rows == 16 ? 0 : rows == 8 ? 1 : rows == 4 ? 2 : -1;
        if (i < 0 || !e.k[i]) break;
        *entry = &e; *slot = i;
        return LINNA_OK;
    }
    set_error("net_stream: %d rows per workgroup", rows);
    return LINNA_ERR_INVALID;
}
static int ns_launch(NsEntry& e, int i, const NsArgs& a, int nblocks, size_t lds_bytes, hipStream_t s) {
    if (!e.attr_set[i]) {
        const int rc = check_hip(hipFuncSetAttribute(reinterpret_cast<const void*>(e.k[i]), hipFuncAttributeMaxDynamicSharedMemorySize, NS_LDS_BYTES),
                                 "hipFuncSetAttribute");
        if (rc != LINNA_OK) return rc;
        e.attr_set[i] = true;
    }
    hipLaunchKernelGGL(e.k[i], dim3(nblocks), dim3(64 * NS_NW), lds_bytes, s, a);
    return check_hip(hipGetLastError(), e.what);
}
static int ns_launch_program(NsVariant v, unsigned flags, const NsArgs& a0, int B, const NsProgram& p, int rows, hipStream_t s, int extra = 0,
                             size_t lds_extra = 0) {
    NsEntry* e = nullptr; int i = 0;
    const int rc = ns_kernel(v, flags, rows, &e, &i);
    if (rc != LINNA_OK) return rc;
#ifdef NS_STAMPS
    NsArgs a = a0;
    a.stamps = getenv("LINNA_FUSED_STAMPS") ? reinterpret_cast<unsigned long long*>(strtoull(getenv("LINNA_FUSED_STAMPS"), nullptr, 16)) : nullptr;
    if (!a.stamps) { set_error("net_stream: NS_STAMPS build needs LINNA_FUSED_STAMPS"); return LINNA_ERR_INVALID; }
#else
    const NsArgs& a = a0;
#endif
    const bool grad = v == NV_GRAD_MLP || v == NV_GRAD2 || v == NV_TRAIN_STEP;
    return ns_launch(*e, i, a, (B + rows - 1) / rows + extra, p.lds_for(rows, grad) + lds_extra, s);
}

__device__ __forceinline__ void as_update(f32x4& P4, const f32x4& G4, f32x4& M4, f32x4& V4, float lr, float wd, float bc1,
                                          float sbc2, float beta1, float beta2, float eps) {
#pragma unroll
    for (int e = 0; e < 4; ++e) {
        const float gi = G4[e];
        float pi = P4[e] * (1.f - lr * wd);
        float mi = M4[e];
        mi = mi + (gi - mi) * (1.f - beta1);
        const float vi = V4[e] * beta2 + (1.f - beta2) * gi * gi;
        const float denom = sqrtf(vi) / sbc2 + eps;
        pi = pi - (lr / bc1) * (mi / denom);
        P4[e] = pi; M4[e] = mi; V4[e] = vi;
    }
}

template <bool BF = false>
__global__ __launch_bounds__(AS_BLOCK) void adamw_streams_kernel(AsArgs a, float* __restrict__ p, const float* __restrict__ g,
                                                            float* __restrict__ m, float* __restrict__ v,
                                                            const float* __restrict__ hyper, float beta1, float beta2, float eps) {
    int ri = 0;
    while (ri + 1 < a.nr && blockIdx.x >= a.r[ri + 1].blk0) ++ri;
// ... 90 lines not shown
    a.T = 1.f;
    for (int i = 0; i < (int)p.seg.size(); ++i) a.seg[i] = p.seg[i];
    return a;
}
static void ns_store_table(NsArgs& a, const NsProgram& p, const NsNet& net, const NsOpBufs* ops, int lo, int hi, bool dx) {
    for (int i = lo; i < hi; ++i) {
        const int op = p.seg_op[i];
        if (op >= net.nl) continue;
        const NsOpBufs& b = ops[op];
        const linna_layer_t& l = net.layers[op];
        a.gn[i] = p.seg_hidden[i] ? l.C : dx ? l.K : l.N;
        if (!dx) { a.gout[i] = p.seg_hidden[i] ? b.t : b.y; a.gld[i] = p.seg_hidden[i] ? b.ldt : b.ldy; }
        else if (p.seg_hidden[i]) { a.gout[i] = b.dt; a.gld[i] = b.lddt; a.gmask[i] = b.t; a.gmld[i] = b.ldt; }
        else { a.gout[i] = b.dprev; a.gld[i] = b.ldp; a.gmask[i] = b.gate; a.gmld[i] = b.ldx; }
    }
}
static bool ns_set_gates(NsArgs& a, const NsGates& g, const NsProgram& p, int rows, size_t* lds_extra) {
    for (int i = 0; i < NS_SEGCAP; ++i) { a.gbit[i] = g.gbit[i]; a.mbit[i] = g.mbit[i]; }
    a.nbw = g.ncols / 32;
    a.bits_off = (int)(g.lds0 / sizeof(float));
    *lds_extra = g.lds - p.lds_for(rows, true);
    return g.ok && g.lds <= (size_t)NS_LDS_BYTES;
}
static void ns_set_input(NsArgs& a, const NsInput& in) {
    a.is_flat = in.is_flat; a.a1 = in.a1; a.a2 = in.a2; a.lg = in.lg; a.xmean = in.xmean; a.xstd = in.xstd;
}
static void ns_set_input_ignored(NsArgs& a, const float* any) {
    a.is_flat = reinterpret_cast<const int*>(any); a.a1 = any; a.a2 = any; a.lg = nullptr; a.xmean = any; a.xstd = any;
}
static void ns_set_grad(NsArgs& a, const NsGrad& gr) {
    a.gscale = gr.gscale; a.Gout = gr.G; a.ldg = gr.ldg;
    const NsLeap& l = gr.leap;
    a.hm_p = l.P; a.hm_ldp = l.ldp; a.hm_q = l.Q; a.hm_mass = l.mass; a.hm_ek = l.ek; a.hm_ed = l.ed; a.hm_eps = l.eps;
}

bool net_stream_takes_plain(NsKind kind, const NsNet& net, const NsOutput& out, const NsRun& r, const NsMove* mv, const NsGrad* gr, int rows,
                            const NsDense* dn) {
    if (kind != NS_SERVE || rows != 16 || mv || gr || dn || !net_stream_serve_plain(-1)) return false;
    if (!net_stream_launch_plain_ok(out.cscale, out.cshift, out.w, out.cpost, r.lnP, r.D, r.TH, r.gate)) return false;
    return ns_program_plain(*ns_program(kind, net.layers, net.nl, net.in_size, dn, rows));
}

int launch_net_stream(NsKind kind, const NsNet& net, const float* packed, const NsRun& r, const NsInput& in, const NsOutput& out,
                      const NsMove* mv, const NsGrad* gr, int rows, const NsDense* dn, hipStream_t s) {
    const bool bf = kind == NS_SERVE_BF16;
    if ((kind == NS_SERVE_DENSE) != (dn != nullptr) || !(kind == NS_SERVE || kind == NS_SERVE_DENSE || bf)) {
        set_error("net_stream: not a serving program"); return LINNA_ERR_INVALID;
    }
    const NsProgramRef pref = ns_program(kind, net.layers, net.nl, net.in_size, dn, rows);
    const NsProgram& p = *pref;
    if ((out.cpost != nullptr) != (out.cshift2 != nullptr) || (out.cpost && (dn || gr))) {
        set_error("net_stream: the exp output map needs cpost and cshift2, and has no dense / gradient program"); return LINNA_ERR_INVALID;
    }
    if (!p.ok) { set_error("net_stream: network not eligible"); return LINNA_ERR_UNSUPPORTED; }
    if (dn && (out.w || gr || out.cscale || out.cshift)) { set_error("net_stream: the dense program carries its own output map and has no fused gradient"); return LINNA_ERR_INVALID; }
    if (mv && (in.nin > 64 || (!out.w && !dn))) { set_error("net_stream: fused sampler moves need <= 64 parameters and a log-likelihood in the launch"); return LINNA_ERR_UNSUPPORTED; }
    if (gr && (!p.grad_ok || !out.w || !r.lnP || !gr->gscale || !gr->G || mv)) { set_error("net_stream: no fused gradient for this network / likelihood"); return LINNA_ERR_UNSUPPORTED; }
    NsArgs a = ns_args(p, packed, r.Z, r.ldz, r.B, in.nin, gr != nullptr);
    ns_set_input(a, in);
    a.cscale = out.cscale; a.cshift = out.cshift; a.w = out.w; a.T = out.T;
    a.cpost = out.cpost; a.cshift2 = out.cshift2;
    a.dense = p.dense ? (dn && dn->factored ? 2 : 1) : 0; a.u_col = p.u_col; a.u_same = p.u_same; a.x0_keep = p.x0_keep;
    a.lnP = r.lnP; a.D = r.D; a.ldd = r.ldd; a.TH = r.TH; a.ldt = r.ldt;
    a.gate = r.gate;
    const unsigned fbf = bf ? NF_BF16 : 0;
    if (mv) {
        a.mv_coords = mv->coords; a.mv_ldc = mv->ldc; a.mv_logp = mv->logp; a.mv_S = mv->S;
        a.mv_cc = mv->cc; a.mv_ldcc = mv->ldcc; a.mv_C = mv->C; a.mv_nc = mv->nc;
        a.mv_seed = mv->seed; a.mv_step = mv->step; a.mv_step_off = mv->step_off; a.mv_stream = mv->stream; a.mv_a = mv->a; a.mv_naccept = mv->naccept;
        a.mv_chain = mv->chain; a.mv_lps = mv->lps;
        a.sl_Z0 = mv->sl_Z0; a.sl_L = mv->sl_L; a.sl_R = mv->sl_R; a.sl_Zt = mv->sl_Zt; a.sl_m = mv->sl_m; a.sl_nt = mv->sl_nt;
        a.sl_seed = mv->sl_seed; a.sl_step = mv->sl_step; a.sl_stream = mv->sl_stream; a.sl_flags = mv->sl_flags;
        if (mv->sb) a.sb = *mv->sb;
        return ns_launch_program(mv->slice ? NV_SLICE : NV_STRETCH, fbf, a, r.B, p, rows, s);
    }
    if (bf && gr) { set_error("net_stream: no bf16 gradient"); return LINNA_ERR_UNSUPPORTED; }
    if (bf) return ns_launch_program(NV_SERVE, NF_BF16, a, r.B, p, rows, s);
    if (gr) {
        ns_set_grad(a, *gr);
        return ns_launch_program(NV_GRAD_MLP, a.hm_p && a.hm_eps ? NF_EPS : 0, a, r.B, p, rows, s);
    }
    if (!net_stream_takes_plain(kind, net, out, r, mv, gr, rows, dn)) return ns_launch_program(NV_SERVE, 0, a, r.B, p, rows, s);
    for (int i = 0; i < a.nseg; ++i) a.seg[i].type |= a.seg[i].ncg_log2 << 8;
#ifdef NS_HAVE_PLACED
    if (net_stream_serve_plain_sched(-1)) return ns_launch_program(NV_SERVE, NF_PLAIN | NF_PLACED, a, r.B, p, rows, s);
#endif
    return ns_launch_program(NV_SERVE, NF_PLAIN, a, r.B, p, rows, s);
}

int launch_net_stream_store(const NsNet& net, const float* packed, const float* X, int ldx, int B, const NsOpBufs* ops,
                            const float* cscale, const float* cshift, int rows, hipStream_t s) {
    const NsProgramRef pref = ns_program(NS_STORE, net.layers, net.nl, net.in_size, nullptr, rows);
    const NsProgram& p = *pref;
    if (!p.ok) { set_error("net_stream: network not eligible"); return LINNA_ERR_UNSUPPORTED; }
    NsArgs a = ns_args(p, packed, X, ldx, B, net.in_size, false);
    ns_set_input_ignored(a, X);
    a.cscale = cscale; a.cshift = cshift;
    ns_store_table(a, p, net, ops, 0, p.nseg_f, false);
    return ns_launch_program(NV_STORE, 0, a, B, p, rows, s);
}


int launch_net_stream_grad2(const NsNet& net, const float* packed, const NsRun& r, const NsInput& in, const NsOutput& out, const NsGrad& gr,
                            int rows, hipStream_t s, bool bf) {
    const NsProgramRef pref = ns_program(bf ? NS_GRAD_INPUT_BF16 : ns_grad_kind(net.layers, net.nl), net.layers, net.nl, net.in_size, nullptr, rows);
    const NsProgram& p = *pref;
    if (!p.ok || !p.dxi_ok) { set_error("net_stream: no forward + dX program for this network"); return LINNA_ERR_UNSUPPORTED; }
    if (!out.w || !r.lnP || !gr.gscale || !gr.G) { set_error("net_stream: the one-launch gradient needs a diagonal covariance"); return LINNA_ERR_INVALID; }
    NsArgs a = ns_args(p, packed, r.Z, r.ldz, r.B, in.nin, true);
    ns_set_input(a, in);
    a.cscale = out.cscale; a.cshift = out.cshift; a.w = out.w; a.T = out.T; a.lnP = r.lnP;
    ns_set_grad(a, gr);
    const NsGates g = ns_gates(p, net.layers, net.nl, rows);
    for (int i = 0; i < (int)p.seg.size(); ++i) if (i >= p.nseg_f || g.gbit[i] >= 0) a.gn[i] = ns_seg_cols(p, net.layers, i);
    size_t lds_extra = 0;
    if (!ns_set_gates(a, g, p, rows, &lds_extra)) {
        set_error(g.ok ? "net_stream: the one-launch gradient's sign bits do not fit the LDS" : "net_stream: a gate of the one-launch gradient has no producer");
        return LINNA_ERR_UNSUPPORTED;
    }
    const unsigned flags = (bf ? NF_BF16 : p.nout > 64 ? NF_WIDE : 0) | (a.hm_p && a.hm_eps ? NF_EPS : 0);
    return ns_launch_program(NV_GRAD2, flags, a, r.B, p, rows, s, 0, lds_extra);
}

int launch_net_stream_grad_dense(const NsNet& net, const float* packed, const NsRun& r, const NsInput& in, float T, const NsGrad& gr,
                                 int rows, const NsDense& dn, hipStream_t s) {
    const NsProgramRef pref = ns_program(NS_GRAD_INPUT_DENSE, net.layers, net.nl, net.in_size, &dn, rows);
    const NsProgram& p = *pref;
    if (!p.ok || !p.dxi_ok || !p.dense || !dn.factored) { set_error("net_stream: no dense forward + dX program for this network"); return LINNA_ERR_UNSUPPORTED; }
    if (!r.lnP || !gr.G) { set_error("net_stream: the dense one-launch gradient needs lnP and G"); return LINNA_ERR_INVALID; }
    NsArgs a = ns_args(p, packed, r.Z, r.ldz, r.B, in.nin, true);
    ns_set_input(a, in);
    a.T = T; a.lnP = r.lnP;
    a.dense = 2; a.u_col = p.u_col; a.u_same = p.u_same;
    ns_set_grad(a, gr);
    a.gscale = nullptr;
    const NsGates g = ns_gates(p, net.layers, net.nl, rows);
    for (int i = 0; i < (int)p.seg.size(); ++i) if (i >= p.nseg_f || g.gbit[i] >= 0) a.gn[i] = ns_seg_cols(p, net.layers, i);
    size_t lds_extra = 0;
    if (!ns_set_gates(a, g, p, rows, &lds_extra)) {
        set_error(g.ok ? "net_stream: the dense one-launch gradient does not fit the LDS of this engine" : "net_stream: a gate of the dense one-launch gradient has no producer");
        return LINNA_ERR_UNSUPPORTED;
    }
    return ns_launch_program(NV_GRAD2, NF_DENSE | (a.hm_p && a.hm_eps ? NF_EPS : 0), a, r.B, p, rows, s, 0, lds_extra);
}

static NsArgs ns_train_args(const NsProgram& p, bool full, const NsNet& net, const float* packed, const NsBatch& b, const NsOpBufs* ops,
                            const NsTrainLoss& L) {
    NsArgs a = ns_args(p, packed, b.X, b.ldx, b.B, net.in_size, full);
    ns_set_input_ignored(a, b.xmean);
    a.lg = b.lg; a.xstd = b.xstd;
    a.dense = p.dense; a.u_col = p.u_col; a.u_same = p.u_same;
    ns_store_table(a, p, net, ops, 0, p.nseg_f, false);
    a.t_rows = b.ROWS; a.t_xb = b.XB; a.t_ldxb = b.ldxb;
    a.t_Y = L.YN; a.t_ldy = L.ldyn;
    a.t_den = L.den; a.t_inv_batch = L.inv_batch; a.t_loss_rows = L.loss_rows; a.t_dP = L.dP; a.t_lddp = L.lddp;
    return a;
}

int launch_net_stream_train(const NsNet& net, const float* packed, const NsBatch& b, const NsOpBufs* ops, const NsTrainLoss& L,
                            const NsDense& dn, int rows, hipStream_t s) {
    const NsProgramRef pref = ns_program(NS_TRAIN_FWD, net.layers, net.nl, net.in_size, &dn, rows);
    const NsProgram& p = *pref;
    if (!p.ok || !p.dense) { set_error("net_stream: network + loss not eligible"); return LINNA_ERR_UNSUPPORTED; }
    const NsArgs a = ns_train_args(p, false, net, packed, b, ops, L);
    return ns_launch_program(NV_TRAIN_FWD, 0, a, b.B, p, rows, s);
}
// ... 38 lines not shown
```

### linna_amd/csrc/net_stream_body.inc

```
    constexpr int NT = NS_NT, NW = NS_NW;
    constexpr int RG = 32;
    constexpr bool SM = ROWS < 16;
    constexpr int RS = SM ? ROWS / 4 : 1;
    constexpr int NQ = SM ? RS : NT;
    constexpr int NACC = SM ? 4 * RS : NT;
#ifdef NS_BODY_SLICE_BF16
    static_assert(BF && !GRAD && STORE == 0 && MOVE == 2, "bf16: the slice evaluation");
#elif defined(NS_BODY_GRAD_BF16)
    static_assert(BF && GRAD && STORE == 2 && MOVE == 0, "bf16: lnP and its gradient in one launch");
#else
    static_assert(!BF || (!GRAD && STORE == 0 && MOVE != 2) || (GRAD && STORE == 3 && MOVE == 0 && ROWS == 4),
                  "bf16: serving, the fused stretch move and the merged training step (4-row engine)");
#endif
    constexpr bool BFT = BF && GRAD && STORE == 3;
    constexpr int AK = BF ? 2 : 1;
    constexpr bool K4 = !SM && !BF && (STORE == 0 || (GRAD && STORE == 2));
    constexpr bool TRB = GRAD && STORE == 3;
    constexpr bool DXE = STORE == 2 || TRB;
    constexpr bool G2 = GRAD && STORE == 2;
    constexpr bool LB = G2;
    constexpr bool LATE_REFILL = true;
#ifdef NS_BODY_HAND
    constexpr bool HAND = true;
    static_assert(PLAIN && !BF && ROWS == 16 && R == 6 && NS_NT == 4 && LATE_REFILL, "the hand-placed step: plain fp32 serving, 16 rows, six slots");
#else
    constexpr bool HAND = false;
#endif
#define NS_HAND_RING \
    "+{v[128:131]}"(Bq[0][0]), "+{v[132:135]}"(Bq[0][1]), "+{v[136:139]}"(Bq[0][2]), "+{v[140:143]}"(Bq[0][3]), \
    "+{v[144:147]}"(Bq[1][0]), "+{v[148:151]}"(Bq[1][1]), "+{v[152:155]}"(Bq[1][2]), "+{v[156:159]}"(Bq[1][3]), \
    "+{v[160:163]}"(Bq[2][0]), "+{v[164:167]}"(Bq[2][1]), "+{v[168:171]}"(Bq[2][2]), "+{v[172:175]}"(Bq[2][3]), \
    "+{v[176:179]}"(Bq[3][0]), "+{v[180:183]}"(Bq[3][1]), "+{v[184:187]}"(Bq[3][2]), "+{v[188:191]}"(Bq[3][3]), \
    "+{v[192:195]}"(Bq[4][0]), "+{v[196:199]}"(Bq[4][1]), "+{v[200:203]}"(Bq[4][2]), "+{v[204:207]}"(Bq[4][3]), \
    "+{v[208:211]}"(Bq[5][0]), "+{v[212:215]}"(Bq[5][1]), "+{v[216:219]}"(Bq[5][2]), "+{v[220:223]}"(Bq[5][3])
#define NS_HAND_A "+{v[224:227]}"(Aq[0][0]), "+{v[228:231]}"(Aq[1][0])
#define NS_HAND_ACC "+{v[232:235]}"(acc[0]), "+{v[236:239]}"(acc[1]), "+{v[240:243]}"(acc[2]), "+{v[244:247]}"(acc[3])
    constexpr bool RNAN = STORE == 1;
    auto relu_f = [](float v) { if constexpr (RNAN) return isnan(v) ? v : fmaxf(v, 0.f); else return fmaxf(v, 0.f); };
    static_assert(ROWS == 16 || ROWS == 8 || ROWS == 4, "rows per workgroup");
    static_assert(R % 2 == 0, "the A double buffer alternates with the ring slot parity");
    extern __shared__ __attribute__((aligned(16))) float smem[];
    const int LD = a.LD, ABUF = ROWS * LD;
    constexpr bool KA = STORE == 3 || STORE == 1 || GRAD;
    const NsArgs* const ka = KA ? reinterpret_cast<const NsArgs*>((const void*)__builtin_amdgcn_kernarg_segment_ptr()) : &a;
    float* const act = smem;
    float* const lbias = smem + 2 * ABUF;
    unsigned* const lbits = reinterpret_cast<unsigned*>(smem + a.bits_off);
    const int nbw = a.nbw;
    const int tid = threadIdx.x, lane = tid & 63;
    const int wave = __builtin_amdgcn_readfirstlane(tid >> 6);
    const int li = lane & 15, kq = lane >> 4;
    const int row0 = blockIdx.x * ROWS;
    if constexpr (!PLAIN) {
        if (a.gate && a.gate[0] == 0) return;
    }
    int mv_rows = a.B;
    if constexpr (MOVE == 2) {
        if (a.mv_C) {
            mv_rows = a.mv_step[0] * a.mv_step_off;
            if (row0 >= mv_rows) return;
        }
    }
    if constexpr ((STORE == 2 && !GRAD) || TRB) {
        if ((a.p_n > 0 || a.p_step) && blockIdx.x == gridDim.x - 1) {
            float* const part = smem;
            float acc0 = 0.f, acc1 = 0.f;
            for (int i = tid; i < a.p_n; i += 1024) acc0 += a.p_rows[i];
            for (int i = tid + 512; i < a.p_n; i += 1024) acc1 += a.p_rows[i];
#pragma unroll
            for (int o = 32; o >= 1; o >>= 1) { acc0 += __shfl_xor(acc0, o, 64); acc1 += __shfl_xor(acc1, o, 64); }
            if (lane == 0) { part[wave] = acc0; part[8 + wave] = acc1; }
            __syncthreads();
            if (tid == 0 && a.p_out) {
                float t = 0.f;
                for (int w = 0; w < 16; ++w) t += part[w];
                a.p_out[0] = t * a.p_scale;
            }
            if (tid == 64 && a.p_step) {
                const int t = ++a.p_step[0];
                a.p_hyper[2] = (float)(1.0 - pow((double)a.p_b1, (double)t));
                a.p_hyper[3] = (float)sqrt(1.0 - pow((double)a.p_b2, (double)t));
            }
            return;
        }
    }
#ifdef NS_STAMPS
    unsigned long long* const lstamp = reinterpret_cast<unsigned long long*>(lbias + ((a.bias_total + 3) & ~3) + 32 + (a.x0_keep ? 1024 : 0)) + wave * 32;
    int nstamp = 0;
#define NS_STAMP() do { const unsigned long long t_ = __builtin_readcyclecounter(); \
        if (lane == 0 && nstamp < 32) lstamp[nstamp] = t_; ++nstamp; } while (0)
#define NS_STAMPS_FLUSH() do { if (lane < 32) a.stamps[((size_t)blockIdx.x * NW + wave) * 32 + lane] = lane < nstamp ? lstamp[lane] : 0ull; } while (0)
#else
#define NS_STAMP() do {} while (0)
#define NS_STAMPS_FLUSH() do {} while (0)
#endif
    NS_STAMP();

    const int prt = tid / RG, pc0 = tid % RG;
    const bool prow = prt < ROWS;
    const int pr = SM ? min(prt, ROWS - 1) : prt;
    int grow = min(row0 + pr, a.B - 1);
    if constexpr (MOVE == 2) {
        if (a.mv_C) grow = a.mv_C[min(row0 + pr, mv_rows - 1)];
    }
    int zsrc = grow;
    float zden = 1.f;
    if constexpr (STORE == 3) {
        zsrc = a.t_rows ? a.t_rows[grow] : grow;
        zden = a.t_den[zsrc];
// ... 90 lines not shown
            }
        } else {
            wgt = a.mv_cc[grow];
        }
#pragma unroll
        for (int i = 0; i < ZPRE; ++i) {
            const int c = min(pc0 + i * RG, nin - 1);
            zr[i] = a.mv_coords[(size_t)wk * a.mv_ldc + c] + wgt * a.Z[(size_t)k * a.ldz + c];
        }
        }
    }
#pragma unroll
    for (int i = 0; i < ZPRE; ++i) {
        const int c = min(pc0 + i * RG, nin - 1);
        if constexpr (MOVE == 0) zr[i] = a.Z[(size_t)(STORE == 3 ? zsrc : grow) * a.ldz + c];
        zfl[i] = a.is_flat[c]; za1[i] = a.a1[c]; za2[i] = a.a2[c];
        zlg[i] = lgp[c]; zxm[i] = a.xmean[c]; zxs[i] = a.xstd[c];
    }
    const int nb4 = (a.bias_total + 3) >> 2;
    const f32x4* const bsrc = reinterpret_cast<const f32x4*>(a.packed + (size_t)NW * a.Gstride * NT * 256);
    constexpr int BMAX = 3;
    f32x4 breg[BMAX];
#pragma unroll
    for (int i = 0; i < BMAX; ++i) {
        const int j = tid + i * 64 * NW;
        breg[i] = bsrc[min(j, nb4 - 1)];
    }
    constexpr int FIN = 2;
    const float* const csp = a.cscale ? a.cscale : a.xmean;
    const float* const ctp = a.cshift ? a.cshift : a.xmean;
    const float* const wtp = a.w ? a.w : a.xmean;
    float fcs[FIN], fct[FIN], fw[FIN], fgs[FIN];
#pragma unroll
    for (int i = 0; i < FIN; ++i) {
        const int cc = min(pc0 + i * RG, nout - 1);
        if constexpr (DGR) {
            fgs[i] = 0.f; fcs[i] = 1.f; fct[i] = 0.f; fw[i] = 0.f;
            continue;
        }
        if constexpr (GRAD && !TRB) fgs[i] = a.gscale[cc]; else fgs[i] = 0.f;
        if constexpr (PLAIN) {
            fcs[i] = a.cscale[cc]; fct[i] = a.cshift[cc]; fw[i] = a.w[cc];
        } else {
        const int c1 = a.cscale ? cc : 0, c2 = a.cshift ? cc : 0, c3 = a.w ? cc : 0;
        const float cs = csp[c1], ct = ctp[c2], ww = wtp[c3];
        fcs[i] = a.cscale ? cs : 1.f; fct[i] = a.cshift ? ct : 0.f; fw[i] = a.w ? ww : 0.f;
        }
    }

    const char* const wbase = reinterpret_cast<const char*>(a.packed) + (size_t)wave * a.Gstride * NS_STEP_B;
    const unsigned wlast = (unsigned)(a.G - 1) * NS_STEP_B;
    unsigned woff = 0;
    const unsigned voff = 16u * (unsigned)lane;
    f32x4 Bq[R][NT];
    auto wload = [&](int t) { return *reinterpret_cast<const f32x4*>(wbase + (size_t)(voff + woff) + t * 1024); };
    auto wadvance = [&]() { woff = min(woff + NS_STEP_B, wlast); };
    constexpr int PRE = NS_PRE < R ? NS_PRE : R;
    auto prefetch = [&](auto Uc) {
        constexpr int U = decltype(Uc)::value;
#pragma unroll
        for (int t = 0; t < NT; ++t) {
            Bq[U][t] = wload(t);
            __builtin_amdgcn_sched_barrier(0);
        }
        wadvance();
    };
#define NS_PF(U, LO, HI) if constexpr (U >= LO && U < HI) prefetch(std::integral_constant<int, U>{});
#define NS_PF_ALL(LO, HI) NS_PF(0, LO, HI) NS_PF(1, LO, HI) NS_PF(2, LO, HI) NS_PF(3, LO, HI) NS_PF(4, LO, HI) NS_PF(5, LO, HI) \
    NS_PF(6, LO, HI) NS_PF(7, LO, HI)
    NS_PF_ALL(0, PRE)
#ifdef NS_STAMPS_FINE
    NS_STAMP();
#endif

    float zz = 0.f;
    float theta[ZPRE];
#pragma unroll
    for (int i = 0; i < ZPRE; ++i) {
        const int c = pc0 + i * RG;
        const bool in = c < nin;
        const float z = in ? zr[i] : 0.f;
        zz += z * z;
        float th = ns_prior_theta(z, zfl[i], za1[i], za2[i]);
        float lt = log10f(th);
        asm volatile("" : "+v"(lt));
        theta[i] = th;
        const float t = (a.lg && zlg[i]) ? lt : th;
        float x = in ? (t - zxm[i]) / zxs[i] : 0.f;
        zz += 0.f * x;
        if constexpr ((STORE == 1 || STORE == 2) && !GRAD) x = z;
        if constexpr (STORE == 3) {
            float lz = log10f(z);
            asm volatile("" : "+v"(lz));
            const float tz = (a.lg && zlg[i]) ? lz : z;
            x = in ? (tz - zxm[i]) / zxs[i] : 0.f;
            if (prow && row0 + pr < a.B && c < a.t_ldxb)
                asm volatile("global_store_dword %0, %1, off" :: "v"(a.t_xb + (size_t)(row0 + pr) * a.t_ldxb + c), "v"(x) : "memory");
        }
        if constexpr (BF) {
            if (prow) {
                if (in) { const float hi = (float)(__bf16)x; act[pr * LD + c] = hi; act[pr * LD + nin + c] = x - hi; }
                else if (c >= 2 * nin && c < kpad0) act[pr * LD + c] = 0.f;
            }
        } else {
            if (c < kpad0 && prow) act[pr * LD + c] = x;
        }
    }
#ifdef NS_STAMPS_FINE
    NS_STAMP();
#endif
    if constexpr ((STORE == 1 || STORE == 2) && !GRAD) {
        const int wcols = kpad0 - ZPRE * RG;
        if (wcols > 0) {
            constexpr int CP = 4;
            for (int base = 0; base < ROWS * wcols; base += CP * 64 * NW) {
                float v[CP];
#pragma unroll
                for (int u = 0; u < CP; ++u) {
                    const int idx = min(base + u * 64 * NW + tid, ROWS * wcols - 1);
                    const int r = idx / wcols, c = ZPRE * RG + idx % wcols;
                    v[u] = a.Z[(size_t)min(row0 + r, a.B - 1) * a.ldz + min(c, nin - 1)];
                }
#pragma unroll
                for (int u = 0; u < CP; ++u) {
                    const int idx = base + u * 64 * NW + tid;
                    if (idx < ROWS * wcols) {
                        const int r = idx / wcols, c = ZPRE * RG + idx % wcols;
                        act[r * LD + c] = c < nin ? v[u] : 0.f;
                    }
                }
            }
        }
    } else
#pragma unroll 1
    for (int c = pc0 + ZPRE * RG; c < kpad0; c += RG) {
        float x = 0.f;
        if (c < nin) {
            const float z = a.Z[(size_t)grow * a.ldz + c];
            zz += z * z;
            const float th = ns_prior_theta(z, a.is_flat[c], a.a1[c], a.a2[c]);
            const float t = (a.lg && a.lg[c]) ? log10f(th) : th;
            x = (t - a.xmean[c]) / a.xstd[c];
            zz += 0.f * x;
            if constexpr ((STORE == 1 || STORE == 2) && !GRAD) x = z;
            if constexpr (STORE == 3) {
                const float zz3 = a.Z[(size_t)zsrc * a.ldz + c];
                x = (((a.lg && a.lg[c]) ? log10f(zz3) : zz3) - a.xmean[c]) / a.xstd[c];
            }
        }
        if constexpr (STORE == 3) {
            if (prow && row0 + pr < a.B && c < a.t_ldxb)
                asm volatile("global_store_dword %0, %1, off" :: "v"(a.t_xb + (size_t)(row0 + pr) * a.t_ldxb + c), "v"(x) : "memory");
        }
        if constexpr (BF) {
            if (prow) {
                if (c < nin) { const float hi = (float)(__bf16)x; act[pr * LD + c] = hi; act[pr * LD + nin + c] = x - hi; }
                else if (c >= 2 * nin) act[pr * LD + c] = 0.f;
            }
        } else {
            if (prow) act[pr * LD + c] = x;
        }
    }
    __builtin_amdgcn_sched_barrier(0);
#ifdef NS_STAMPS_FINE
    NS_STAMP();
#endif
    NS_PF_ALL(PRE, (LATE_REFILL ? R - 1 : R))
#undef NS_PF_ALL
#undef NS_PF
#pragma unroll
    for (int o = RG / 2; o >= 1; o >>= 1) zz += __shfl_xor(zz, o, 64);
#pragma unroll
    for (int i = 0; i < BMAX; ++i) {
        const int j = tid + i * 64 * NW;
        if (j < nb4) reinterpret_cast<f32x4*>(lbias)[j] = breg[i];
    }
    int* const lsrc = reinterpret_cast<int*>(lbias + ((a.bias_total + 3) & ~3));
    float* const lden = reinterpret_cast<float*>(lsrc + 16);
    if constexpr (STORE == 3) {
        if (prow && pc0 == 0) { lsrc[pr] = zsrc; lden[pr] = zden; }
    }
    float* const lx0 = lden + 16;
    if constexpr (!PLAIN) {
    if (a.x0_keep && prow) {
#pragma unroll
        for (int i = 0; i < ZPRE; ++i) {
            const int c = pc0 + i * RG;
            if constexpr (BF) lx0[pr * 64 + c] = c < nin ? act[pr * LD + c] + act[pr * LD + nin + c] : 0.f;
            else lx0[pr * 64 + c] = (c < kpad0) ? act[pr * LD + c] : 0.f;
        }
    }
    }
    asm volatile("s_waitcnt lgkmcnt(0)" ::: "memory");
    __builtin_amdgcn_s_barrier();
    asm volatile("" ::: "memory");
    NS_STAMP();

    if constexpr (HAND) {
#pragma unroll
        for (int t = 0; t < NT; ++t) Bq[R - 1][t] = f32x4{0.f, 0.f, 0.f, 0.f};
        asm volatile("" : NS_HAND_RING :: "memory");
    }
    const uint32_t act_lds = (uint32_t)(uintptr_t)(__attribute__((address_space(3))) void*)act;
    f32x4 acc[NACC];
    f32x4 Aq[2][AK];
    const int sm_arow = (4 * ((lane >> 2) & 3) + (lane & 3)) % ROWS, sm_achunk = lane >> 4;
    int si = 0, pass = 0, P = 0, kleft;
    int s_type, s_steps, s_passes, s_bias, s_dst, s_relu, s_kslice, s_zext, s_ncgl, s_mstore = 0, s_mapply = 0, s_x0col = 0, s_x0n = 0, s_kcl = 0;
    unsigned* const lmask = reinterpret_cast<unsigned*>(lbias + ((a.bias_total + 3) & ~3));
    float lnp_grad = 0.f;
    float* s_gout = nullptr; int s_gld = 0, s_gn = 0;
    const float* s_gmask = nullptr; int s_gmld = 0;
    int s_gbit = -1, s_mbit = -1;
    auto gstore = [&](float* p, float v) { asm volatile("global_store_dword %0, %1, off" :: "v"(p), "v"(v) : "memory"); };
    uint32_t ap;
    auto a_read = [&](f32x4* dst) {
        if constexpr (HAND) {
            if (dst == Aq[0]) asm volatile("ds_read_b128 %0, %1" : "={v[224:227]}"(Aq[0][0]) : "v"(ap) : "memory");
            else asm volatile("ds_read_b128 %0, %1" : "={v[228:231]}"(Aq[1][0]) : "v"(ap) : "memory");
        } else
        asm volatile("ds_read_b128 %0, %1" : "=v"(dst[0]) : "v"(ap) : "memory");
        if constexpr (BF) asm volatile("ds_read_b128 %0, %1 offset:16" : "=v"(dst[1]) : "v"(ap) : "memory");
        if constexpr (BFT) ap += si == a.nseg_f - 1 ? 64 : 64 * AK;
        else ap += 64 * AK;
    };
    auto load_seg = [&]() {
        const NsSeg S = ka->seg[__builtin_amdgcn_readfirstlane(si)];
        s_type = S.type; kleft = s_steps = S.steps; s_passes = S.passes; s_bias = S.bias_off;
        s_dst = S.dst_col; s_relu = S.relu; s_kslice = S.kslice; s_zext = S.zext; s_ncgl = S.ncg_log2; s_x0col = S.x0_col; s_x0n = S.x0_n;
        if constexpr (GRAD) { s_mstore = S.mask_store; s_mapply = S.mask_apply; }
        if constexpr (STORE) { const int j = __builtin_amdgcn_readfirstlane(si); s_gout = ka->gout[j]; s_gld = ka->gld[j]; s_gn = ka->gn[j]; }
        if constexpr (DXE) { const int j = __builtin_amdgcn_readfirstlane(si); s_gmask = ka->gmask[j]; s_gmld = ka->gmld[j]; }
        if constexpr (LB) { const int j = __builtin_amdgcn_readfirstlane(si); s_gbit = ka->gbit[j]; s_mbit = ka->mbit[j]; }
    };
    NsSeg nxp;
    auto plain_request = [&]() { nxp = ka->seg[__builtin_amdgcn_readfirstlane(min(si + 1, nseg - 1))]; };
    auto plain_take = [&](const NsSeg& X) {
        s_type = X.type & 255; s_ncgl = X.type >> 8; kleft = s_steps = X.steps; s_passes = X.passes; s_bias = X.bias_off;
        s_dst = X.dst_col; s_relu = X.relu; s_kslice = X.kslice; s_zext = X.zext;
    };
    auto begin_run = [&]() {
        const int arow = SM ? sm_arow : li, ak = AK * (SM ? 4 * sm_achunk : 4 * kq);
#pragma unroll
        for (int t = 0; t < NACC; ++t) acc[t] = f32x4{0.f, 0.f, 0.f, 0.f};
        if (s_type == NS_WIDE) {
            const int blk = !PLAIN && s_zext < 0 ? (pass ? 15 - wave : wave) : 8 * pass + wave;
            if constexpr (SM) {
                const float b = lbias[s_bias + 64 * blk + lane];
#pragma unroll
                for (int r = 0; r < RS; ++r) acc[4 * r] = f32x4{b, b, b, b};
            } else {
#pragma unroll
                for (int t = 0; t < NT; ++t) {
                    const float b = lbias[s_bias + 16 * (4 * blk + t) + li];
                    acc[t] = f32x4{b, b, b, b};
                }
            }
            if (!PLAIN && s_zext < 0) kleft = s_steps - 4 * blk;
            ap = act_lds + 4u * (uint32_t)(P * ABUF + arow * LD + ak + (PLAIN ? 0 : s_zext < 0 ? 64 * blk : (pass ? s_kslice : 0)));
        } else {
            ap = act_lds + 4u * (uint32_t)(P * ABUF + arow * LD + ak + (wave >> s_ncgl) * s_kslice);
        }
        if constexpr (BFT) {
            if (si == a.nseg_f - 1) ap -= 4u * (uint32_t)(ak / 2);
        }
        if constexpr (HAND) asm volatile("s_nop 3" : NS_HAND_ACC);
    };
    auto lds_barrier = [&]() {
        asm volatile("s_waitcnt lgkmcnt(0)" ::: "memory");
        __builtin_amdgcn_s_barrier();
        asm volatile("" ::: "memory");
    };
    if constexpr (PLAIN) {
        asm volatile("" :: "s"(seg_warm));
        plain_take(ka->seg[0]); begin_run(); a_read(Aq[0]); plain_request();
    }
    else {
    load_seg();
    begin_run();
    a_read(Aq[0]);
    }

    auto step = [&](auto Uc, auto Refill) {
        constexpr int U = decltype(Uc)::value;
        constexpr bool refill = decltype(Refill)::value;
        constexpr int RU = LATE_REFILL ? (U + R - 1) % R : U;
        if constexpr (HAND) {
            constexpr int BU = 128 + 16 * U, BR = 128 + 16 * RU, AC = 224 + 4 * (U & 1), AN = 224 + 4 * ((U + 1) & 1);
            constexpr int TW = refill ? 0 : 4 * U;
#define NS_HM(t, s) "v_mfma_f32_16x16x4_f32 v[232+4*" #t ":235+4*" #t "], v[%[ac]+" #s "], v[%[bu]+4*" #t "+" #s "], v[232+4*" #t ":235+4*" #t "]\n\t"
#define NS_HL(t, off) "global_load_dwordx4 v[%[ru]+4*" #t ":%[ru]+4*" #t "+3], %[vo], %[sb] offset:" #off "\n\t"
#define NS_HAND_TEXT(HEAD, L0, L1, L2, L3) HEAD \
            "s_waitcnt lgkmcnt(0)\n\t" \
            "s_waitcnt vmcnt(%[w0])\n\t" \
            NS_HM(0, 0) "ds_read_b128 v[%[an]:%[an]+3], %[ap]\n\t" \
            "s_waitcnt vmcnt(%[w1])\n\t" \
            NS_HM(1, 0) \
            NS_HM(0, 1) L0 \
            NS_HM(1, 1) \
            NS_HM(0, 2) L1 \
            NS_HM(1, 2) \
            NS_HM(0, 3) L2 \
            NS_HM(1, 3) \
            "s_waitcnt vmcnt(%[w2])\n\t" \
            NS_HM(2, 0) L3 \
            "s_waitcnt vmcnt(%[w3])\n\t" \
            NS_HM(3, 0) \
            NS_HM(2, 1) "v_add_u32 %[ap], 64, %[ap]\n\t" \
            NS_HM(3, 1) NS_HM(2, 2) NS_HM(3, 2) NS_HM(2, 3) NS_HM(3, 3)
            if constexpr (refill) {
                const char* const sb = wbase + woff;
#ifdef NS_HAND_PHASE4
#define NS_HAND_HEAD ".p2align 3\n\ts_nop 0\n\t"
#else
#define NS_HAND_HEAD ".p2align 3\n\t"
#endif
                if constexpr (U == 0)
                    asm volatile(NS_HAND_TEXT(NS_HAND_HEAD, NS_HL(0, 0), NS_HL(1, 1024), NS_HL(2, 2048), NS_HL(3, 3072))
                                 : NS_HAND_RING, NS_HAND_A, NS_HAND_ACC, [ap] "+v"(ap)
                                 : [vo] "v"(voff), [sb] "s"(sb), [bu] "n"(BU), [ru] "n"(BR), [ac] "n"(AC), [an] "n"(AN),
                                   [w0] "n"(19), [w1] "n"(18), [w2] "n"(20), [w3] "n"(20) : "memory");
                else
                    asm volatile(NS_HAND_TEXT("", NS_HL(0, 0), NS_HL(1, 1024), NS_HL(2, 2048), NS_HL(3, 3072))
                                 : NS_HAND_RING, NS_HAND_A, NS_HAND_ACC, [ap] "+v"(ap)
                                 : [vo] "v"(voff), [sb] "s"(sb), [bu] "n"(BU), [ru] "n"(BR), [ac] "n"(AC), [an] "n"(AN),
                                   [w0] "n"(19), [w1] "n"(18), [w2] "n"(20), [w3] "n"(20) : "memory");
                wadvance();
            } else {
                asm volatile(NS_HAND_TEXT("", "", "", "", "")
                             : NS_HAND_RING, NS_HAND_A, NS_HAND_ACC, [ap] "+v"(ap)
                             : [bu] "n"(BU), [ac] "n"(AC), [an] "n"(AN),
                               [w0] "n"(19 - TW), [w1] "n"(18 - TW), [w2] "n"(17 - TW), [w3] "n"(16 - TW) : "memory");
            }
#undef NS_HAND_TEXT
#undef NS_HAND_HEAD
#undef NS_HL
#undef NS_HM
        } else {
        if constexpr (BF) asm volatile("s_waitcnt lgkmcnt(0)" : "+v"(Aq[U & 1][0]), "+v"(Aq[U & 1][AK - 1]) :: "memory");
        else asm volatile("s_waitcnt lgkmcnt(0)" : "+v"(Aq[U & 1][0]) :: "memory");
        a_read(Aq[(U + 1) & 1]);
        const f32x4 av = Aq[U & 1][0];
        if constexpr (BF) {
            bf16x8 ab;
#pragma unroll
            for (int e = 0; e < 4; ++e) { ab[e] = (__bf16)Aq[U & 1][0][e]; ab[4 + e] = (__bf16)Aq[U & 1][AK - 1][e]; }
            if constexpr (SM) {
                auto bf_small = [&]() {
                    const s16x4 alo = __builtin_bit_cast(s16x4, __builtin_shufflevector(ab, ab, 0, 1, 2, 3));
                    const s16x4 ahi = __builtin_bit_cast(s16x4, __builtin_shufflevector(ab, ab, 4, 5, 6, 7));
#define NS_B4(r, c, h, A4) acc[4 * (r) + (c)] = __builtin_amdgcn_mfma_f32_4x4x4bf16_1k(A4, \
                __builtin_bit_cast(s16x4, __builtin_shufflevector(__builtin_bit_cast(bf16x8, Bq[U][c]), __builtin_bit_cast(bf16x8, Bq[U][c]), \
                                                                  4 * (h), 4 * (h) + 1, 4 * (h) + 2, 4 * (h) + 3)), acc[4 * (r) + (c)], 4, 4 * (c) + (r), 0);
#define NS_B4R(r, h, A4) NS_B4(r, 0, h, A4) NS_B4(r, 1, h, A4) NS_B4(r, 2, h, A4) NS_B4(r, 3, h, A4)
                    NS_B4R(0, 0, alo)
                    if constexpr (RS > 1) { NS_B4R(1, 0, alo) }
                    NS_B4R(0, 1, ahi)
                    if constexpr (RS > 1) { NS_B4R(1, 1, ahi) }
#undef NS_B4R
#undef NS_B4
                };
                if constexpr (BFT) {
                    if (si == a.nseg_f - 1) {
#define NS_M4(r, c, e) acc[4 * (r) + (c)] = __builtin_amdgcn_mfma_f32_4x4x1f32(av[e], Bq[U][c][e], acc[4 * (r) + (c)], 4, 4 * (c) + (r), 0);
#define NS_M4R(r, e) NS_M4(r, 0, e) NS_M4(r, 1, e) NS_M4(r, 2, e) NS_M4(r, 3, e)
#pragma unroll
                        for (int e = 0; e < 4; ++e) {
                            NS_M4R(0, e)
                            if constexpr (RS > 1) { NS_M4R(1, e) }
                        }
#undef NS_M4R
#undef NS_M4
                    } else {
                        bf_small();
                    }
                } else {
                    bf_small();
                }
                if constexpr (refill) {
#pragma unroll
                    for (int t = 0; t < NT; ++t) Bq[RU][t] = wload(t);
                }
            } else {
#pragma unroll
                for (int h = 0; h < NT; h += 2) {
                    acc[h] = __builtin_amdgcn_mfma_f32_16x16x32_bf16(ab, __builtin_bit_cast(bf16x8, Bq[U][h]), acc[h], 0, 0, 0);
                    acc[h + 1] = __builtin_amdgcn_mfma_f32_16x16x32_bf16(ab, __builtin_bit_cast(bf16x8, Bq[U][h + 1]), acc[h + 1], 0, 0, 0);
                    if constexpr (refill) {
                        Bq[RU][h] = wload(h);
                        Bq[RU][h + 1] = wload(h + 1);
                    }
                }
            }
        } else if constexpr (SM) {
#define NS_M4(r, c, e) acc[4 * (r) + (c)] = __builtin_amdgcn_mfma_f32_4x4x1f32(av[e], Bq[U][c][e], acc[4 * (r) + (c)], 4, 4 * (c) + (r), 0);
#define NS_M4R(r, e) NS_M4(r, 0, e) NS_M4(r, 1, e) NS_M4(r, 2, e) NS_M4(r, 3, e)
#pragma unroll
            for (int e = 0; e < 4; ++e) {
                NS_M4R(0, e)
                if constexpr (RS > 1) { NS_M4R(1, e) }
            }
#undef NS_M4R
#undef NS_M4
            if constexpr (refill) {
#pragma unroll
                for (int t = 0; t < NT; ++t) Bq[RU][t] = wload(t);
            }
        } else {
#pragma unroll
            for (int h = 0; h < NT; h += 2) {
#pragma unroll
                for (int s = 0; s < 4; ++s) {
                    acc[h] = __builtin_amdgcn_mfma_f32_16x16x4f32(av[s], Bq[U][h][s], acc[h], 0, 0, 0);
                    acc[h + 1] = __builtin_amdgcn_mfma_f32_16x16x4f32(av[s], Bq[U][h + 1][s], acc[h + 1], 0, 0, 0);
                }
                if constexpr (refill) {
                    Bq[RU][h] = wload(h);
                    Bq[RU][h + 1] = wload(h + 1);
                }
            }
        }
        if constexpr (refill) wadvance();
        }
        if (--kleft == 0) {
            if constexpr (HAND) asm volatile("s_nop 15" : NS_HAND_ACC);
            const int nxi = __builtin_amdgcn_readfirstlane(min(si + 1, nseg - 1));
            const NsSeg NX = ka->seg[nxi];
            float* nx_gout = nullptr; int nx_gld = 0, nx_gn = 0;
            const float* nx_gmask = nullptr; int nx_gmld = 0;
            if constexpr (STORE) { nx_gout = ka->gout[nxi]; nx_gld = ka->gld[nxi]; nx_gn = ka->gn[nxi]; }
            if constexpr (DXE) { nx_gmask = ka->gmask[nxi]; nx_gmld = ka->gmld[nxi]; }
            int nx_gbit = -1, nx_mbit = -1;
            if constexpr (LB) { nx_gbit = ka->gbit[nxi]; nx_mbit = ka->mbit[nxi]; }
            const int cur_steps = s_steps;
            auto take_seg = [&](const NsSeg& X) {
                s_type = X.type; s_steps = X.steps; s_passes = X.passes; s_bias = X.bias_off;
                s_dst = X.dst_col; s_relu = X.relu; s_kslice = X.kslice; s_zext = X.zext; s_ncgl = X.ncg_log2; s_x0col = X.x0_col; s_x0n = X.x0_n;
                if constexpr (K4) s_kcl = X.kcl;
                if constexpr (GRAD) { s_mstore = X.mask_store; s_mapply = X.mask_apply; }
                kleft = X.steps;
            };
            auto take_next = [&]() {
                if constexpr (PLAIN) { plain_take(nxp); return; }
                take_seg(NX);
                if constexpr (STORE) { s_gout = nx_gout; s_gld = nx_gld; s_gn = nx_gn; }
                if constexpr (DXE) { s_gmask = nx_gmask; s_gmld = nx_gmld; }
                if constexpr (LB) { s_gbit = nx_gbit; s_mbit = nx_mbit; }
            };
            f32x4 sdw[2][NT];
            bool side_next = false;
            if constexpr (K4 && !PLAIN) {
#pragma unroll
                for (int s2 = 0; s2 < 2; ++s2)
#pragma unroll
                    for (int t = 0; t < NT; ++t) sdw[s2][t] = f32x4{0.f, 0.f, 0.f, 0.f};
                if (NX.type == NS_SIDE && si + 1 < nseg && (s_type != NS_WIDE || pass + 1 == s_passes)) {
                    side_next = true;
                    const char* const sb = reinterpret_cast<const char*>(a.packed + NX.side_off) + (size_t)wave * NX.steps * NS_STEP_B + voff;
#pragma unroll
                    for (int t = 0; t < NT; ++t)
                        asm volatile("global_load_dwordx4 %0, %1, off" : "=v"(sdw[0][t]) : "v"(sb + t * 1024) : "memory");
                    if (NX.steps > 1) {
#pragma unroll
                        for (int t = 0; t < NT; ++t)
                            asm volatile("global_load_dwordx4 %0, %1, off" : "=v"(sdw[1][t]) : "v"(sb + NS_STEP_B + t * 1024) : "memory");
                    }
                }
            }
            bool seg_done = true;
#ifdef NS_STAMPS_FINE
            const bool fine = si >= NS_STAMPS_FINE && si < NS_STAMPS_FINE + 4;
            if (fine) NS_STAMP();
#endif
            if constexpr (SM) {
#pragma unroll
                for (int q = 0; q < NQ; ++q) acc[q] = (acc[4 * q] + acc[4 * q + 1]) + (acc[4 * q + 2] + acc[4 * q + 3]);
            }
#define fin acc
#define q_row(q, e) (SM ? 4 * (q) + (e) : 4 * kq + (e))
#define q_col(q) (SM ? lane : 16 * (q) + li)
            if (s_type == NS_WIDE) {
                float* const nxt = act + (P ^ 1) * ABUF + s_dst + (!PLAIN && s_zext < 0 ? 64 * (pass ? 15 - wave : wave) : 512 * pass + 64 * wave);
                float ty[NQ][4];
                if constexpr (STORE == 3) {
                    if (si == nlast) {
#pragma unroll
                        for (int t = 0; t < NQ; ++t) {
                            const int dc = min(512 * pass + 64 * wave + q_col(t), nout - 1);
#pragma unroll
                            for (int e = 0; e < 4; ++e) {
                                const float* py = a.t_Y + (size_t)lsrc[q_row(t, e)] * a.t_ldy + dc;
                                asm volatile("global_load_dword %0, %1, off" : "=v"(ty[t][e]) : "v"(py) : "memory");
                            }
                        }
#pragma unroll
                        for (int t = 0; t < NQ; ++t)
                            asm volatile("s_waitcnt vmcnt(0)" : "+v"(ty[t][0]), "+v"(ty[t][1]), "+v"(ty[t][2]), "+v"(ty[t][3]) :: "memory");
                    }
                }
                unsigned long long gw[SM ? NQ : 1][4];
                if constexpr (LB) {
                    if (s_mbit >= 0) {
                        const int cw = 512 * pass + 64 * wave, w0 = (s_mbit + cw) >> 5;
                        const bool mine = cw < ((s_gn + 63) & ~63);
#pragma unroll
                        for (int t = 0; t < (SM ? NQ : 1); ++t)
#pragma unroll
// ... 363 lines not shown
                            const f32x4 f1 = kc4 ? af1 : af0, f2 = kc4 ? af2 : kc1 ? af0 : af1, f3 = kc4 ? af3 : kc1 ? af0 : af1;
#pragma unroll
                            for (int e = 0; e < 4; ++e) {
                                acc[0] = __builtin_amdgcn_mfma_f32_16x16x4f32(af0[e], sdw[s2][0][e], acc[0], 0, 0, 0);
                                acc[1] = __builtin_amdgcn_mfma_f32_16x16x4f32(f1[e], sdw[s2][1][e], acc[1], 0, 0, 0);
                            }
#pragma unroll
                            for (int e = 0; e < 4; ++e) {
                                acc[2] = __builtin_amdgcn_mfma_f32_16x16x4f32(f2[e], sdw[s2][2][e], acc[2], 0, 0, 0);
                                acc[3] = __builtin_amdgcn_mfma_f32_16x16x4f32(f3[e], sdw[s2][3][e], acc[3], 0, 0, 0);
                            }
                        }
                    }
                    int treal = NT;
                    if (kc4) { acc[0] = (acc[0] + acc[1]) + (acc[2] + acc[3]); treal = 1; }
                    else if (!kc1) { acc[0] = acc[0] + acc[2]; acc[1] = acc[1] + acc[3]; treal = 2; }
                    float* const part = act + (P ^ 1) * ABUF;
                    constexpr int PW = ROWS * 64;
#pragma unroll
                    for (int t = 0; t < NT; ++t)
                        if (t < treal) {
#pragma unroll
                            for (int e = 0; e < 4; ++e) part[wave * PW + (4 * kq + e) * 64 + ((16 * t + li) ^ (16 * kq))] = acc[t][e];
                        }
#ifdef NS_STAMPS_FINE
                    if (fine) NS_STAMP();
#endif
                    lds_barrier();
#ifdef NS_STAMPS_FINE
                    if (fine) NS_STAMP();
#endif
                    {
                        float* const cur = act + P * ABUF + pr * LD + s_dst;
                        const int ncol = 16 * treal, sw = 16 * (pr >> 2);
                        for (int c = 4 * pc0; c < s_zext; c += 4 * RG) {
                            f32x4 v = f32x4{0.f, 0.f, 0.f, 0.f};
                            if (c < ncol) {
                                const float* src = part + pr * 64 + (c ^ sw);
                                constexpr int CH = LB ? 4 : NW;
                                const f32x4 b = *reinterpret_cast<const f32x4*>(lbias + s_bias + c);
#pragma unroll
                                for (int k0 = 0; k0 < NW; k0 += CH) {
                                    f32x4 x[CH];
#pragma unroll
                                    for (int kp = 0; kp < CH; ++kp) x[kp] = *reinterpret_cast<const f32x4*>(src + (k0 + kp) * PW);
#pragma unroll
                                    for (int kp = 0; kp < CH; ++kp) v += x[kp];
                                }
                                v += b;
                                if (s_relu) v = f32x4{fmaxf(v[0], 0.f), fmaxf(v[1], 0.f), fmaxf(v[2], 0.f), fmaxf(v[3], 0.f)};
                            }
                            if constexpr (LB) {
                                const bool mine = c < ((s_gn + 63) & ~63);
                                if (s_mbit >= 0) {
                                    const unsigned nib = mine ? (lbits[pr * nbw + ((s_mbit + c) >> 5)] >> (c & 31)) & 0xFu : 0u;
#pragma unroll
                                    for (int e = 0; e < 4; ++e) v[e] = ((nib >> e) & 1u) ? v[e] : 0.f;
                                }
                                *reinterpret_cast<f32x4*>(cur + c) = v;
                                if (s_gbit >= 0) {
                                    unsigned w32 = ((v[0] > 0.f ? 1u : 0u) | (v[1] > 0.f ? 2u : 0u) | (v[2] > 0.f ? 4u : 0u) | (v[3] > 0.f ? 8u : 0u)) << (c & 31);
                                    w32 |= __shfl_xor(w32, 1, 64); w32 |= __shfl_xor(w32, 2, 64); w32 |= __shfl_xor(w32, 4, 64);
                                    if ((pc0 & 7) == 0 && mine) lbits[pr * nbw + ((s_gbit + c) >> 5)] = w32;
                                }
                            } else {
                                *reinterpret_cast<f32x4*>(cur + c) = v;
                            }
                        }
                    }
#ifdef NS_STAMPS_FINE
                    if (fine) { asm volatile("s_waitcnt lgkmcnt(0)" ::: "memory"); NS_STAMP(); }
#endif
                    lds_barrier();
                    NS_STAMP();
                    ++si;
                    const int n2i = __builtin_amdgcn_readfirstlane(min(si, nseg - 1));
                    const NsSeg N2 = ka->seg[n2i];
                    take_seg(N2);
                    if constexpr (LB) { s_gbit = ka->gbit[n2i]; s_mbit = ka->mbit[n2i]; s_gn = ka->gn[n2i]; }
                }
            }
            if (si < nseg) {
                begin_run();
                a_read(Aq[(U + 1) & 1]);
                if constexpr (PLAIN) { if (seg_done) plain_request(); }
            }
#ifdef NS_STAMPS_FINE
            if (fine) { asm volatile("s_waitcnt lgkmcnt(0)" ::: "memory"); NS_STAMP(); }
#endif
        }
    };
    using T_ = std::true_type; using F_ = std::false_type;
#define NS_STEP(U, RF) if constexpr (U < R) step(std::integral_constant<int, U>{}, RF{});
    const int ngroups = a.G / R, rem = a.G - ngroups * R;
#pragma unroll 1
    for (int it = 0; it < ngroups; ++it) {
        NS_STEP(0, T_) NS_STEP(1, T_) NS_STEP(2, T_) NS_STEP(3, T_) NS_STEP(4, T_) NS_STEP(5, T_) NS_STEP(6, T_) NS_STEP(7, T_)
    }
#define NS_TAIL(U) if constexpr (U < R - 1) { if (rem > U) step(std::integral_constant<int, U>{}, F_{}); }
    NS_TAIL(0) NS_TAIL(1) NS_TAIL(2) NS_TAIL(3) NS_TAIL(4) NS_TAIL(5) NS_TAIL(6)
#undef NS_STEP
#undef NS_TAIL
    if constexpr (BF) asm volatile("s_waitcnt lgkmcnt(0)" : "+v"(Aq[0][0]), "+v"(Aq[0][AK - 1]), "+v"(Aq[1][0]), "+v"(Aq[1][AK - 1]) :: "memory");
    else asm volatile("s_waitcnt lgkmcnt(0)" : "+v"(Aq[0][0]), "+v"(Aq[1][0]) :: "memory");
    NS_STAMP();

    if constexpr (((STORE == 1 || STORE == 2) && !GRAD) || TRB) { NS_STAMPS_FLUSH(); return; }
    if constexpr (STORE == 3) {
        const float* const F = act + P * ABUF + pr * LD;
        const bool rok = prow && row0 + pr < a.B;
        const float* const Dv = a.u_same ? F : act + (P ^ 1) * ABUF + pr * LD;
        const float* const Uv = a.u_same ? F + a.u_col : F;
        float chi = 0.f;
        for (int c = pc0; c < nout; c += RG) chi += Dv[c] * Uv[c];
#pragma unroll
        for (int o = RG / 2; o >= 1; o >>= 1) chi += __shfl_xor(chi, o, 64);
        if (rok && pc0 == 0) a.t_loss_rows[row0 + pr] = chi / lden[pr];
        {
            constexpr int TPR = 64 * NW / ROWS;
            const int fr = tid / TPR, fc = tid % TPR;
            if (row0 + fr < a.B) {
                const float* const Fr = act + P * ABUF + fr * LD;
                const float* const Dr = a.u_same ? Fr : act + (P ^ 1) * ABUF + fr * LD;
                const float* const Ur = a.u_same ? Fr + a.u_col : Fr;
                const float dr = lden[fr];
                for (int c = fc; c < a.t_lddp; c += TPR) {
                    float g = 0.f;
                    if (c < nout) {
                        const bool masked = __float_as_uint(Dr[c]) == 0x80000000u;
                        g = masked ? 0.f : (-2.f * Ur[c]) * a.t_inv_batch / dr;
                    }
                    a.t_dP[(size_t)(row0 + fr) * a.t_lddp + c] = g;
                }
            }
        }
        NS_STAMP();
        NS_STAMPS_FLUSH();
        return;
    }
    if constexpr (GRAD) {
        const float* const F = act + P * ABUF + pr * LD;
        const bool rok = prow && row0 + pr < a.B;
        if (rok) {
            float hm_ek = a.hm_ek, hm_ed = a.hm_ed;
            if constexpr (EPS) { const float e = a.hm_eps[row0 + pr]; hm_ek *= e; hm_ed *= e; }
#pragma unroll
            for (int j = 0; j < ZPRE; ++j) {
                const int c = pc0 + j * RG;
                if (c < nin) {
                    float g = F[c] / zxs[j];
                    if (a.lg && zlg[j]) g = g / (theta[j] * 2.30258509299404568f);
                    const float z = zr[j];
                    const float dth = zfl[j] ? za2[j] * (expf(-0.5f * z * z) * 0.398942280401432678f) : za2[j];
                    const float gz = g * dth - z;
                    a.Gout[(size_t)(row0 + pr) * a.ldg + c] = gz;
                    if (a.hm_p) {
                        float* const pp = a.hm_p + (size_t)(row0 + pr) * a.hm_ldp + c;
                        float pm = *pp;
                        if (a.hm_ek != 0.f) { pm += hm_ek * gz; *pp = pm; }
                        if (a.hm_ed != 0.f) a.hm_q[(size_t)(row0 + pr) * a.ldz + c] = z + hm_ed * (pm / a.hm_mass[c]);
                    }
                }
            }
            if (pc0 == 0) a.lnP[row0 + pr] = isnan(lnp_grad) ? -INFINITY : lnp_grad;
        }
        if constexpr (STORE == 2) { NS_STAMP(); NS_STAMPS_FLUSH(); }
        return;
    }
    {
        const float* const F = act + P * ABUF + pr * LD;
        const bool rok = prow && row0 + pr < a.B;
        float chi = 0.f;
        auto column = [&](int c, float cs, float ct, float ww) {
            float d = F[c] * cs + ct;
            if (!PLAIN && a.cpost) d = expf(d) * a.cpost[c] + a.cshift2[c];
            if (!PLAIN && a.D && rok) a.D[(size_t)(row0 + pr) * a.ldd + c] = isnan(zz) ? zz : d;
            chi += (d * ww) * d;
        };
        if (!PLAIN && a.dense) {
            const float* const Dv = a.u_same ? F : act + (P ^ 1) * ABUF + pr * LD;
            const float* const U = a.u_same ? F + a.u_col : F;
            const bool fac = a.dense == 2;
            for (int c = pc0; c < nout; c += RG) {
                const float d = Dv[c];
                if (a.D && rok) a.D[(size_t)(row0 + pr) * a.ldd + c] = isnan(zz) ? zz : d;
// ... 55 lines not shown
```

### linna_amd/nn.py

```python
import collections
import ctypes as C
import math

import numpy as np
import torch

from . import _lib

__all__ = ["ChtoModelv2", "ChtoModelv2_linear", "ChtoModelsimple", "MLP", "MLP4x512", "ResBlock_batchnorm"]


def _hidden(out_size):
    return 1000 if out_size > 30 else max(32, int(out_size * 32))


def _xavier_uniform(shape):
    bound = math.sqrt(3.0) * math.sqrt(2.0 / float(shape[0] + shape[1]))
    return torch.empty(shape, dtype=torch.float32).uniform_(-bound, bound)


def _consume(n):
    if n > 0:
        torch.empty(int(n), dtype=torch.float32).uniform_()

# ... 307 lines not shown
        ops.append(_Op(L, "layer7", h6, self.out_size, relu=1))
        ops.append(_Op(L, "layer8", self.out_size, self.out_size, relu=0))
        return ops


class ChtoModelsimple(ChtoModelv2):
    channel = 4
    wide_layer6 = False


class ChtoModelv2_linear(ChtoModelv2):

    def _build_ops(self):
        ops = ChtoModelv2._build_ops(self)
        ops.append(_Op(_lib.OP_INSKIP, "linearlayer", self.in_size, self.out_size, alpha=1e-3))
        return ops

    def _post_init(self):
        self._view(self._flat, "linearlayer.bias").zero_()
        self._view(self._flat, "linearlayer.weight").fill_(1e-5)


class MLP(_Emulator):

    def __init__(self, in_size, out_size, linearmodel=None, docpu=False, width=512, depth=4):
        self.width, self.depth = int(width), int(depth)
        _Emulator.__init__(self, in_size, out_size, linearmodel, docpu)

    def _build_ops(self):
        ops, k = [], self.in_size
        for i in range(self.depth):
            ops.append(_Op(_lib.OP_LINEAR, "layer%d" % (i + 1), k, self.width, relu=1))
            k = self.width
        ops.append(_Op(_lib.OP_LINEAR, "layer%d" % (self.depth + 1), k, self.out_size, relu=0))
        return ops


MLP4x512 = MLP


class ResBlock_batchnorm(object):

    def __init__(self, in_size, channel, out_size):
        self.in_size, self.channel, self.out_size = in_size, channel, out_size
        self.op = _Op(_lib.OP_RESBLOCK, "block", in_size, out_size, C=channel)


def program_layers(model):
    arr = _lib.sized_array(_lib.Layer, len(model.ops))
    nxt = [4096]

    def fake(n):
        p = nxt[0]
        nxt[0] += 16 * ((int(n) + 3) // 4 + 1)
        return C.c_void_p(p)
    for i, op in enumerate(model.ops):
        L = arr[i]
        L.op, L.K, L.C, L.N, L.relu, L.alpha = op.op, op.K, op.C, op.N, op.relu, op.alpha
        if op.op == _lib.OP_RESBLOCK:
            L.W1, L.b1, L.W2, L.b2 = fake(op.C * op.K), fake(op.C), fake(op.N * op.C), fake(op.N)
            if op.K != op.N:
                L.Ws = fake(op.N * op.K)
        else:
            L.W, L.b = fake(op.N * op.K), fake(op.N)
    return arr


def describe_program(model, rows=16, dense_nout=0):
    arr = program_layers(model)
    buf = C.create_string_buffer(8192)
    n = _lib.load().linna_program_describe(arr, len(model.ops), model.in_size, int(rows), int(dense_nout), buf, len(buf))
    if n < 0:
        _lib.check(n)
    return n, buf.value.decode()


def program_is_plain(model, rows=16, dense_nout=0):
    n = _lib.load().linna_program_plain(program_layers(model), len(model.ops), model.in_size, int(rows), int(dense_nout))
    if n < 0:
        _lib.check(n)
    return bool(n)


def describe_grad_bf16_program(model, rows=16):
    arr = program_layers(model)
    buf = C.create_string_buffer(8192)
    n = _lib.load().linna_program_describe_grad_bf16(arr, len(model.ops), model.in_size, int(rows), buf, len(buf))
    if n < 0:
        _lib.check(n)
    return n, buf.value.decode()


def describe_grad_dense_program(model, rows=16, tri=2):
    arr = program_layers(model)
    buf = C.create_string_buffer(8192)
    n = _lib.load().linna_program_describe_grad_dense(arr, len(model.ops), model.in_size, model.out_size, int(tri), int(rows), buf, len(buf))
    if n < 0:
        _lib.check(n)
    return n, buf.value.decode()
```

Measured before the change: 76.27 million evals/s.

## Add trimmed hand-placed serving kernel skipping dead MFMA tiles and log10

Adds a new plain-serving kernel variant, enabled by default, that runs each layer segment as a run-length loop over hand-written assembly step texts. Per-segment metadata folds the live output-column count and live K-slice count into the segment type. This lets waves skip MFMA tiles for padded columns (the T3 text for 33-wide outputs) and shrink the final partial K step (the S1 text). It also skips log10f in the prior map when log parameters are off, and replaces the unrolled six-slot step loop with a scalar-branch jump table over ring slots. This cuts wasted matrix work on the 33-wide input and output layers, at the cost of extra scalar branching and fragile hand-placed waitcnt and register scheduling.

```diff
diff --git a/include/linna_hip.h b/include/linna_hip.h
--- a/include/linna_hip.h
+++ b/include/linna_hip.h
@@ -167,6 +167,8 @@
 int linna_dense_tri(int mode);
 int linna_serve_plain(int on);
 int linna_serve_plain_sched(int hand);
+int linna_serve_plain_trim(int on);
+int linna_program_trim(const linna_layer_t* layers, int nlayers, int in_size, int rows, char* buf, size_t n);
 int linna_program_plain(const linna_layer_t* layers, int nlayers, int in_size, int rows, int dense_nout);
 int linna_logprob_serve_plain(linna_logprob_t* lp, int B, int* out);
 int linna_logprob_grad_launches(linna_logprob_t* lp, int B, int* out);
diff --git a/linna_amd/_lib.py b/linna_amd/_lib.py
--- a/linna_amd/_lib.py
+++ b/linna_amd/_lib.py
@@ -133,6 +133,8 @@
     "linna_dense_tri": (_I, [_I]),
     "linna_serve_plain": (_I, [_I]),
     "linna_serve_plain_sched": (_I, [_I]),
+    "linna_serve_plain_trim": (_I, [_I]),
+    "linna_program_trim": (_I, [_V, _I, _I, _I, _V, C.c_size_t]),
     "linna_program_plain": (_I, [_V, _I, _I, _I, _I]),
     "linna_logprob_serve_plain": (_I, [_V, _I, _V]),
     "linna_logprob_grad_launches": (_I, [_V, _I, _V]),
@@ -364,6 +366,13 @@
     return prev
 
 
+def serve_plain_trim(on=-1):
+    prev = load().linna_serve_plain_trim(int(on))
+    if prev < 0:
+        check(prev)
+    return prev
+
+
 def serve_plain(on=-1):
     prev = load().linna_serve_plain(int(on))
     if prev < 0:
diff --git a/linna_amd/csrc/api.hip b/linna_amd/csrc/api.hip
--- a/linna_amd/csrc/api.hip
+++ b/linna_amd/csrc/api.hip
@@ -1159,6 +1159,15 @@
     if (hand < -1 || hand > 1) { set_error("linna_serve_plain_sched: %d (-1 query, 0 or 1)", hand); return LINNA_ERR_INVALID; }
     return net_stream_serve_plain_sched(hand);
 } LINNA_CATCH_INT
+int linna_serve_plain_trim(int on) try {
+    if (on < -1 || on > 1) { set_error("linna_serve_plain_trim: %d (-1 query, 0 or 1)", on); return LINNA_ERR_INVALID; }
+    return net_stream_serve_plain_trim(on);
+} LINNA_CATCH_INT
+int linna_program_trim(const linna_layer_t* layers, int nlayers, int in_size, int rows, char* buf, size_t n) try {
+    if (!layers || nlayers < 1 || !buf || !n) { set_error("program_trim: bad arguments"); return LINNA_ERR_INVALID; }
+    TRY(check_layers(layers, nlayers, "program_trim"));
+    return net_stream_trim_describe(layers, nlayers, in_size, rows, buf, n);
+} LINNA_CATCH_INT
 int linna_program_plain(const linna_layer_t* layers, int nlayers, int in_size, int rows, int dense_nout) try {
     if (!layers || nlayers < 1) { set_error("program_plain: bad arguments"); return LINNA_ERR_INVALID; }
     TRY(check_layers(layers, nlayers, "program_plain"));
diff --git a/linna_amd/csrc/common.h b/linna_amd/csrc/common.h
--- a/linna_amd/csrc/common.h
+++ b/linna_amd/csrc/common.h
@@ -318,6 +318,8 @@
 int net_stream_describe(NsKind kind, const linna_layer_t* layers, int nl, int in_size, const NsDense* dn, int rows, char* buf, size_t n);
 int net_stream_serve_plain(int on);
 int net_stream_serve_plain_sched(int hand);
+int net_stream_serve_plain_trim(int on);
+int net_stream_trim_describe(const linna_layer_t* layers, int nl, int in_size, int rows, char* buf, size_t n);
 bool net_stream_program_plain(NsKind kind, const linna_layer_t* layers, int nl, int in_size, const NsDense* dn, int rows);
 bool net_stream_launch_plain_ok(bool cscale, bool cshift, bool w, bool cexp, bool lnP, bool D, bool TH, bool gate);
 struct NsNet { const linna_layer_t* layers; int nl, in_size; };
diff --git a/linna_amd/csrc/net_program.h b/linna_amd/csrc/net_program.h
--- a/linna_amd/csrc/net_program.h
+++ b/linna_amd/csrc/net_program.h
@@ -65,6 +65,9 @@
 NsProgramRef ns_program(NsKind kind, const linna_layer_t* layers, int nl, int in_size, const NsDense* dn, int rows);
 
 bool ns_program_plain(const NsProgram& p);
+int ns_trim_slive(const NsProgram& p, int i, int kp);
+int ns_trim_tlive(const NsProgram& p, int i, int pass, int wave);
+int ns_trim_fold(const NsProgram& p, int i);
 int ns_seg_cols(const NsProgram& p, const linna_layer_t* layers, int i);
 struct NsGates {
     int gbit[NS_SEGCAP], mbit[NS_SEGCAP];
diff --git a/linna_amd/csrc/net_program.hip b/linna_amd/csrc/net_program.hip
--- a/linna_amd/csrc/net_program.hip
+++ b/linna_amd/csrc/net_program.hip
@@ -437,6 +437,62 @@
 int net_stream_serve_plain(int on) { return on < 0 ? g_serve_plain.load() : g_serve_plain.exchange(on ? 1 : 0); }
 static std::atomic<int> g_serve_plain_sched{1};
 int net_stream_serve_plain_sched(int hand) { return hand < 0 ? g_serve_plain_sched.load() : g_serve_plain_sched.exchange(hand ? 1 : 0); }
+static std::atomic<int> g_serve_plain_trim{1};
+int net_stream_serve_plain_trim(int on) { return on < 0 ? g_serve_plain_trim.load() : g_serve_plain_trim.exchange(on ? 1 : 0); }
+
+int ns_trim_slive(const NsProgram& p, int i, int kp) {
+    const NsSeg& g = p.seg[i];
+    const NsPackSeg& q = p.pack[i];
+    if (q.Kb) return 4;
+    const int k0 = (g.type == NS_SPLIT ? kp * g.kslice : 0) + 16 * (g.steps - 1);
+    return std::min(std::max(q.Ka - k0, 0), 4);
+}
+int ns_trim_tlive(const NsProgram& p, int i, int pass, int wave) {
+    const NsSeg& g = p.seg[i];
+    const int c0 = 64 * (g.type == NS_WIDE ? 8 * pass + wave : wave & ((1 << g.ncg_log2) - 1));
+    return std::min(std::max((p.pack[i].N - c0 + 15) / 16, 0), 4);
+}
+static int ns_trim_slive_folded(const NsProgram& p, int i) {
+    const int nkp = p.seg[i].type == NS_SPLIT ? NS_NW >> p.seg[i].ncg_log2 : 1;
+    const int s0 = ns_trim_slive(p, i, 0);
+    for (int kp = 1; kp < nkp; ++kp)
+        if (ns_trim_slive(p, i, kp) != s0) return 4;
+#ifdef NS_TRIM_NO_S1
+    return 4;
+#endif
+    return s0 ? s0 : 4;
+}
+int ns_trim_fold(const NsProgram& p, int i) { return (std::min(p.pack[i].N, 4095) << 12) | ((ns_trim_slive_folded(p, i) - 1) << 24); }
+
+int net_stream_trim_describe(const linna_layer_t* layers, int nl, int in_size, int rows, char* buf, size_t n) {
+    const NsProgramRef pref = ns_program(NS_SERVE, layers, nl, in_size, nullptr, rows);
+    const NsProgram& p = *pref;
+    const bool plain = rows == 16 && ns_program_plain(p);
+    std::string out = plain ? "plain" : "not plain";
+    char line[96];
+    snprintf(line, sizeof line, " G %d nseg_f %d\n", p.G, p.nseg_f);
+    out += line;
+    for (int i = 0; plain && i < p.nseg_f; ++i) {
+        const NsSeg& g = p.seg[i];
+        const int nkp = g.type == NS_SPLIT ? NS_NW >> g.ncg_log2 : 1;
+        snprintf(line, sizeof line, "%s steps %d passes %d slive", g.type == NS_WIDE ? "WIDE" : "SPLIT", g.steps, g.passes);
+        out += line;
+        for (int kp = 0; kp < nkp; ++kp) { snprintf(line, sizeof line, " %d", ns_trim_slive(p, i, kp)); out += line; }
+        out += " tlive";
+        for (int w = 0; w < g.passes * NS_NW; ++w) { snprintf(line, sizeof line, " %d", ns_trim_tlive(p, i, w / NS_NW, w % NS_NW)); out += line; }
+        out += " text";
+        const int fold = ns_trim_fold(p, i), N = (fold >> 12) & 4095;
+        const bool s1 = ((fold >> 24) & 3) == 0;
+        for (int w = 0; w < g.passes * NS_NW; ++w) {
+            const int c0 = 64 * (g.type == NS_WIDE ? w : (w % NS_NW) & ((1 << g.ncg_log2) - 1));
+            const bool t3 = N - c0 > 32 && N - c0 <= 48;
+            out += t3 && s1 ? " T3+S1" : t3 ? " T3" : s1 ? " S1" : " full";
+        }
+        out += "\n";
+    }
+    if (buf && n) snprintf(buf, n, "%s", out.c_str());
+    return plain ? p.nseg_f : 0;
+}
 
 int ns_seg_cols(const NsProgram& p, const linna_layer_t* layers, int i) {
     if (p.seg_op[i] >= p.nops) return p.nout;
diff --git a/linna_amd/csrc/net_stream.hip b/linna_amd/csrc/net_stream.hip
--- a/linna_amd/csrc/net_stream.hip
+++ b/linna_amd/csrc/net_stream.hip
@@ -223,6 +223,17 @@
 #include "net_stream_body.inc"
 #undef NS_BODY_HAND
 }
+#define NS_HAVE_TRIM 1
+template <int R>
+__global__ __launch_bounds__(64 * NS_NW, 1) void net_stream_trim_kernel(NsArgs a) {
+    constexpr int MOVE = 0, STORE = 0, ROWS = 16;
+    constexpr bool GRAD = false, BF = false, EPS = false, PLAIN = true, WOUT = false, DGR = false;
+#define NS_BODY_HAND
+#define NS_BODY_TRIM
+#include "net_stream_body.inc"
+#undef NS_BODY_TRIM
+#undef NS_BODY_HAND
+}
 #endif
 template <int R, int MOVE, bool GRAD, int STORE, int ROWS, bool BF>
 __global__ __launch_bounds__(64 * NS_NW, 1) void net_stream_train_bf16_kernel(NsArgs a) {
@@ -300,7 +311,8 @@
 
 typedef void (*NsKernel)(NsArgs);
 enum NsVariant { NV_SERVE, NV_STRETCH, NV_SLICE, NV_GRAD_MLP, NV_GRAD2, NV_STORE, NV_DX, NV_TRAIN_FWD, NV_TRAIN_STEP };
-enum : unsigned { NF_BF16 = 1, NF_EPS = 2, NF_WIDE = 4, NF_PLAIN = 8, NF_PLACED = 16, NF_DENSE = 32 };
+enum : unsigned { NF_BF16 = 1, NF_EPS = 2, NF_WIDE = 4, NF_PLAIN = 8, NF_PLACED = 16, NF_DENSE = 32,
+                  NF_TRIM = 64 };
 struct NsEntry { NsVariant v; unsigned flags; NsKernel k[3]; const char* what; const char* stamps_lacks; bool attr_set[3]; };
 #define NS_ENGINES(K, MOVE, GRAD, STORE, ...) \
     {K<NS_R, MOVE, GRAD, STORE, 16, __VA_ARGS__>, K<NS_R, MOVE, GRAD, STORE, 8, __VA_ARGS__>, K<NS_R, MOVE, GRAD, STORE, 4, __VA_ARGS__>}
@@ -310,6 +322,9 @@
     {NV_SERVE, NF_PLAIN, {net_stream_plain_kernel<NS_R>, nullptr, nullptr}, "net_stream plain launch"},
 #ifdef NS_HAVE_PLACED
     {NV_SERVE, NF_PLAIN | NF_PLACED, {net_stream_placed_kernel<NS_R>, nullptr, nullptr}, "net_stream plain launch (hand-placed step)"},
+#endif
+#ifdef NS_HAVE_TRIM
+    {NV_SERVE, NF_PLAIN | NF_PLACED | NF_TRIM, {net_stream_trim_kernel<NS_R>, nullptr, nullptr}, "net_stream plain launch (hand-placed step, trimmed)"},
 #endif
     {NV_STRETCH, 0, NS_ENGINES(net_stream_kernel, 1, false, 0, false), "net_stream launch"},
     {NV_STRETCH, NF_BF16, NS_ENGINES(net_stream_kernel, 1, false, 0, true), "net_stream launch"},
@@ -566,6 +581,12 @@
     }
     if (!net_stream_takes_plain(kind, net, out, r, mv, gr, rows, dn)) return ns_launch_program(NV_SERVE, 0, a, r.B, p, rows, s);
     for (int i = 0; i < a.nseg; ++i) a.seg[i].type |= a.seg[i].ncg_log2 << 8;
+#ifdef NS_HAVE_TRIM
+    if (net_stream_serve_plain_sched(-1) && net_stream_serve_plain_trim(-1)) {
+        for (int i = 0; i < a.nseg; ++i) a.seg[i].type |= ns_trim_fold(p, i);
+        return ns_launch_program(NV_SERVE, NF_PLAIN | NF_PLACED | NF_TRIM, a, r.B, p, rows, s);
+    }
+#endif
 #ifdef NS_HAVE_PLACED
     if (net_stream_serve_plain_sched(-1)) return ns_launch_program(NV_SERVE, NF_PLAIN | NF_PLACED, a, r.B, p, rows, s);
 #endif
diff --git a/linna_amd/csrc/net_stream_body.inc b/linna_amd/csrc/net_stream_body.inc
--- a/linna_amd/csrc/net_stream_body.inc
+++ b/linna_amd/csrc/net_stream_body.inc
@@ -25,6 +25,12 @@
     static_assert(PLAIN && !BF && ROWS == 16 && R == 6 && NS_NT == 4 && LATE_REFILL, "the hand-placed step: plain fp32 serving, 16 rows, six slots");
 #else
     constexpr bool HAND = false;
+#endif
+#ifdef NS_BODY_TRIM
+    constexpr bool TRIM = true;
+    static_assert(HAND, "the trimmed step texts are hand-placed ones");
+#else
+    constexpr bool TRIM = false;
 #endif
 #define NS_HAND_RING \
     "+{v[128:131]}"(Bq[0][0]), "+{v[132:135]}"(Bq[0][1]), "+{v[136:139]}"(Bq[0][2]), "+{v[140:143]}"(Bq[0][3]), \
@@ -281,8 +287,11 @@
         const float z = in ? zr[i] : 0.f;
         zz += z * z;
         float th = ns_prior_theta(z, zfl[i], za1[i], za2[i]);
-        float lt = log10f(th);
-        asm volatile("" : "+v"(lt));
+        float lt = th;
+        if (!TRIM || a.lg) {
+            lt = log10f(th);
+            asm volatile("" : "+v"(lt));
+        }
         theta[i] = th;
         const float t = (a.lg && zlg[i]) ? lt : th;
         float x = in ? (t - zxm[i]) / zxs[i] : 0.f;
@@ -406,6 +415,7 @@
     const int sm_arow = (4 * ((lane >> 2) & 3) + (lane & 3)) % ROWS, sm_achunk = lane >> 4;
     int si = 0, pass = 0, P = 0, kleft;
     int s_type, s_steps, s_passes, s_bias, s_dst, s_relu, s_kslice, s_zext, s_ncgl, s_mstore = 0, s_mapply = 0, s_x0col = 0, s_x0n = 0, s_kcl = 0;
+    int s_N = 0, s_sl1 = 0, s_trim = 0, s_sel = 0, s_tx = 0, s_n = 0;
     unsigned* const lmask = reinterpret_cast<unsigned*>(lbias + ((a.bias_total + 3) & ~3));
     float lnp_grad = 0.f;
     float* s_gout = nullptr; int s_gld = 0, s_gn = 0;
@@ -435,7 +445,9 @@
     NsSeg nxp;
     auto plain_request = [&]() { nxp = ka->seg[__builtin_amdgcn_readfirstlane(min(si + 1, nseg - 1))]; };
     auto plain_take = [&](const NsSeg& X) {
-        s_type = X.type & 255; s_ncgl = X.type >> 8; kleft = s_steps = X.steps; s_passes = X.passes; s_bias = X.bias_off;
+        s_type = X.type & 255; kleft = s_steps = X.steps; s_passes = X.passes; s_bias = X.bias_off;
+        if constexpr (TRIM) { s_ncgl = (X.type >> 8) & 15; s_N = (X.type >> 12) & 4095; s_sl1 = ((X.type >> 24) & 3) == 0 ? 2 : 0; }
+        else s_ncgl = X.type >> 8;
         s_dst = X.dst_col; s_relu = X.relu; s_kslice = X.kslice; s_zext = X.zext;
     };
     auto begin_run = [&]() {
@@ -464,6 +476,10 @@
             if (si == a.nseg_f - 1) ap -= 4u * (uint32_t)(ak / 2);
         }
         if constexpr (HAND) asm volatile("s_nop 3" : NS_HAND_ACC);
+        if constexpr (TRIM) {
+            const int c0 = 64 * (s_type == NS_WIDE ? 8 * pass + wave : wave & ((1 << s_ncgl) - 1));
+            s_trim = __builtin_amdgcn_readfirstlane(s_sl1 | (s_N - c0 > 32 && s_N - c0 <= 48 ? 1 : 0));
+        }
     };
     auto lds_barrier = [&]() {
         asm volatile("s_waitcnt lgkmcnt(0)" ::: "memory");
@@ -480,15 +496,21 @@
     a_read(Aq[0]);
     }
 
-    auto step = [&](auto Uc, auto Refill) {
+    auto step = [&](auto Uc, auto Refill, auto Txc) {
         constexpr int U = decltype(Uc)::value;
         constexpr bool refill = decltype(Refill)::value;
+        constexpr int TX = decltype(Txc)::value;
+        static_assert(TX == 0 || (TRIM && refill), "parts of a step: the trimmed launch, whose steps always refill");
+        if constexpr (TX != 4) {
         constexpr int RU = LATE_REFILL ? (U + R - 1) % R : U;
         if constexpr (HAND) {
             constexpr int BU = 128 + 16 * U, BR = 128 + 16 * RU, AC = 224 + 4 * (U & 1), AN = 224 + 4 * ((U + 1) & 1);
             constexpr int TW = refill ? 0 : 4 * U;
-#define NS_HM(t, s) "v_mfma_f32_16x16x4_f32 v[232+4*" #t ":235+4*" #t "], v[%[ac]+" #s "], v[%[bu]+4*" #t "+" #s "], v[232+4*" #t ":235+4*" #t "]\n\t"
-#define NS_HL(t, off) "global_load_dwordx4 v[%[ru]+4*" #t ":%[ru]+4*" #t "+3], %[vo], %[sb] offset:" #off "\n\t"
+#define NS_XM(AC, BU, t, s) "v_mfma_f32_16x16x4_f32 v[232+4*" #t ":235+4*" #t "], v[" #AC "+" #s "], v[" #BU "+4*" #t "+" #s "], v[232+4*" #t ":235+4*" #t "]\n\t"
+#define NS_XLS(SB, RU, t, off) "global_load_dwordx4 v[" #RU "+4*" #t ":" #RU "+4*" #t "+3], %[vo], " #SB " offset:" #off "\n\t"
+#define NS_HM(t, s) NS_XM(%[ac], %[bu], t, s)
+#define NS_HL(t, off) NS_XLS(%[sb], %[ru], t, off)
+#define NS_XL(RU, t, off) NS_XLS(vcc, RU, t, off)
 #define NS_HAND_TEXT(HEAD, L0, L1, L2, L3) HEAD \
             "s_waitcnt lgkmcnt(0)\n\t" \
             "s_waitcnt vmcnt(%[w0])\n\t" \
@@ -507,6 +529,67 @@
             NS_HM(3, 0) \
             NS_HM(2, 1) "v_add_u32 %[ap], 64, %[ap]\n\t" \
             NS_HM(3, 1) NS_HM(2, 2) NS_HM(3, 2) NS_HM(2, 3) NS_HM(3, 3)
+#define NS_XHEAD(AC, AN, BU) \
+            "s_waitcnt lgkmcnt(0)\n\t" \
+            "s_waitcnt vmcnt(19)\n\t" \
+            NS_XM(AC, BU, 0, 0) "ds_read_b128 v[" #AN ":" #AN "+3], %[ap]\n\t" \
+            "s_waitcnt vmcnt(18)\n\t" \
+            NS_XM(AC, BU, 1, 0)
+#define NS_XHALF(AC, BU, RU) \
+            NS_XM(AC, BU, 0, 1) NS_XL(RU, 0, 0) \
+            NS_XM(AC, BU, 1, 1) \
+            NS_XM(AC, BU, 0, 2) NS_XL(RU, 1, 1024) \
+            NS_XM(AC, BU, 1, 2) \
+            NS_XM(AC, BU, 0, 3) NS_XL(RU, 2, 2048) \
+            NS_XM(AC, BU, 1, 3) \
+            "s_waitcnt vmcnt(20)\n\t" \
+            NS_XM(AC, BU, 2, 0) NS_XL(RU, 3, 3072) NS_XADV
+#define NS_XADV \
+            "s_add_u32 %[wo], %[wo], 0x1000\n\t" "s_min_u32 %[wo], %[wo], %[wl]\n\t" \
+            "s_add_u32 vcc_lo, %[wbl], %[wo]\n\t" "s_addc_u32 vcc_hi, %[wbh], 0\n\t"
+#define NS_XADD "v_add_u32 %[ap], 64, %[ap]\n\t"
+#define NS_XFULL(AC, AN, BU, RU) NS_XHEAD(AC, AN, BU) NS_XHALF(AC, BU, RU) \
+            "s_waitcnt vmcnt(20)\n\t" \
+            NS_XM(AC, BU, 3, 0) \
+            NS_XM(AC, BU, 2, 1) NS_XADD \
+            NS_XM(AC, BU, 3, 1) NS_XM(AC, BU, 2, 2) NS_XM(AC, BU, 3, 2) NS_XM(AC, BU, 2, 3) NS_XM(AC, BU, 3, 3)
+#define NS_XT3(AC, AN, BU, RU) NS_XHEAD(AC, AN, BU) NS_XHALF(AC, BU, RU) \
+            NS_XM(AC, BU, 2, 1) NS_XADD \
+            NS_XM(AC, BU, 2, 2) NS_XM(AC, BU, 2, 3)
+#define NS_XS1(AC, AN, BU, RU) NS_XHEAD(AC, AN, BU) \
+            "s_waitcnt vmcnt(17)\n\t" \
+            NS_XM(AC, BU, 2, 0) NS_XL(RU, 0, 0) \
+            "s_waitcnt vmcnt(17)\n\t" \
+            NS_XM(AC, BU, 3, 0) NS_XL(RU, 1, 1024) NS_XL(RU, 2, 2048) NS_XL(RU, 3, 3072) NS_XADV \
+            NS_XADD
+#define NS_XRING(L, TEXT) \
+            "s_cmp_eq_u32 %[sel], 1\n\t" "s_cbranch_scc1 " #L "1f\n\t" "s_cmp_eq_u32 %[sel], 2\n\t" "s_cbranch_scc1 " #L "2f\n\t" \
+            "s_cmp_eq_u32 %[sel], 3\n\t" "s_cbranch_scc1 " #L "3f\n\t" "s_cmp_eq_u32 %[sel], 4\n\t" "s_cbranch_scc1 " #L "4f\n\t" \
+            "s_cmp_eq_u32 %[sel], 5\n\t" "s_cbranch_scc1 " #L "5f\n\t" \
+            ".p2align 3\n" \
+            #L "0:\n\t" TEXT(224, 228, 128, 208) NS_XCNT #L "1:\n\t" TEXT(228, 224, 144, 128) NS_XCNT \
+            #L "2:\n\t" TEXT(224, 228, 160, 144) NS_XCNT #L "3:\n\t" TEXT(228, 224, 176, 160) NS_XCNT \
+            #L "4:\n\t" TEXT(224, 228, 192, 176) NS_XCNT #L "5:\n\t" TEXT(228, 224, 208, 192) NS_XCNT \
+            "s_branch " #L "0b\n"
+#define NS_XCNT "s_add_u32 %[n], %[n], -1\n\t" "s_cmp_eq_u32 %[n], 0\n\t" "s_cbranch_scc1 99f\n"
+#define NS_XONE(U, AC, AN, BU, RU) \
+            "s_cmp_lg_u32 %[sel], " #U "\n\t" "s_cbranch_scc1 1" #U "f\n\t" NS_XS1(AC, AN, BU, RU) "s_branch 99f\n" "1" #U ":\n\t"
+            if constexpr (TX == 5) {
+                static_assert(NS_STEP_B == 0x1000, "the stream advance in the text");
+                const unsigned wbl = __builtin_amdgcn_readfirstlane((unsigned)(uintptr_t)wbase);
+                const unsigned wbh = __builtin_amdgcn_readfirstlane((unsigned)((uintptr_t)wbase >> 32));
+                asm volatile("s_add_u32 vcc_lo, %[wbl], %[wo]\n\t" "s_addc_u32 vcc_hi, %[wbh], 0\n\t"
+                             "s_cmp_eq_u32 %[n], 0\n\t" "s_cbranch_scc1 60f\n\t"
+                             "s_cmp_lg_u32 %[tx], 0\n\t" "s_cbranch_scc1 58f\n\t"
+                             NS_XRING(4, NS_XFULL)
+                             "58:\n\t" NS_XRING(5, NS_XT3)
+                             "60:\n\t"
+                             NS_XONE(0, 224, 228, 128, 208) NS_XONE(1, 228, 224, 144, 128) NS_XONE(2, 224, 228, 160, 144)
+                             NS_XONE(3, 228, 224, 176, 160) NS_XONE(4, 224, 228, 192, 176) NS_XONE(5, 228, 224, 208, 192) "99:\n\t"
+                             : NS_HAND_RING, NS_HAND_A, NS_HAND_ACC, [ap] "+v"(ap), [wo] "+s"(woff), [n] "+s"(s_n)
+                             : [vo] "v"(voff), [wbl] "s"(wbl), [wbh] "s"(wbh), [wl] "s"(wlast),
+                               [sel] "s"(__builtin_amdgcn_readfirstlane(s_sel)), [tx] "s"(__builtin_amdgcn_readfirstlane(s_tx)) : "memory", "scc", "vcc");
+            } else
             if constexpr (refill) {
                 const char* const sb = wbase + woff;
 #ifdef NS_HAND_PHASE4
@@ -532,9 +615,22 @@
                                [w0] "n"(19 - TW), [w1] "n"(18 - TW), [w2] "n"(17 - TW), [w3] "n"(16 - TW) : "memory");
             }
 #undef NS_HAND_TEXT
+#undef NS_XONE
+#undef NS_XCNT
+#undef NS_XRING
+#undef NS_XS1
+#undef NS_XT3
+#undef NS_XFULL
+#undef NS_XADD
+#undef NS_XADV
+#undef NS_XHALF
+#undef NS_XHEAD
 #undef NS_HAND_HEAD
 #undef NS_HL
 #undef NS_HM
+#undef NS_XL
+#undef NS_XLS
+#undef NS_XM
         } else {
         if constexpr (BF) asm volatile("s_waitcnt lgkmcnt(0)" : "+v"(Aq[U & 1][0]), "+v"(Aq[U & 1][AK - 1]) :: "memory");
         else asm volatile("s_waitcnt lgkmcnt(0)" : "+v"(Aq[U & 1][0]) :: "memory");
@@ -621,7 +717,10 @@
         }
         if constexpr (refill) wadvance();
         }
-        if (--kleft == 0) {
+        }
+        bool run_end = TX == 4;
+        if constexpr (TX == 0) run_end = --kleft == 0;
+        if (run_end) {
             if constexpr (HAND) asm volatile("s_nop 15" : NS_HAND_ACC);
             const int nxi = __builtin_amdgcn_readfirstlane(min(si + 1, nseg - 1));
             const NsSeg NX = ka->seg[nxi];
@@ -1151,6 +1250,11 @@
             }
             if (si < nseg) {
                 begin_run();
+                if constexpr (TX == 4) {
+                    asm volatile("ds_read_b128 v[224:227], %2\n\tds_read_b128 v[228:231], %2"
+                                 : "={v[224:227]}"(Aq[0][0]), "={v[228:231]}"(Aq[1][0]) : "v"(ap) : "memory");
+                    ap += 64;
+                } else
                 a_read(Aq[(U + 1) & 1]);
                 if constexpr (PLAIN) { if (seg_done) plain_request(); }
             }
@@ -1160,16 +1264,32 @@
         }
     };
     using T_ = std::true_type; using F_ = std::false_type;
-#define NS_STEP(U, RF) if constexpr (U < R) step(std::integral_constant<int, U>{}, RF{});
+    using X0_ = std::integral_constant<int, 0>;
+#define NS_STEP(U, RF) if constexpr (U < R) step(std::integral_constant<int, U>{}, RF{}, X0_{});
     const int ngroups = a.G / R, rem = a.G - ngroups * R;
+    if constexpr (TRIM) {
+        const int G = a.G;
+        int g = 0;
+#pragma unroll 1
+        while (g < G) {
+            const int n = __builtin_amdgcn_readfirstlane((s_trim & 2) ? kleft - 1 : kleft);
+            s_n = n;
+            s_tx = s_trim & 1;
+            step(X0_{}, T_{}, std::integral_constant<int, 5>{});
+            const int done = n ? n : 1;
+            g += done; kleft -= done; s_sel = (s_sel + done) % R;
+            if (kleft == 0) step(X0_{}, T_{}, std::integral_constant<int, 4>{});
+        }
+    } else {
 #pragma unroll 1
     for (int it = 0; it < ngroups; ++it) {
         NS_STEP(0, T_) NS_STEP(1, T_) NS_STEP(2, T_) NS_STEP(3, T_) NS_STEP(4, T_) NS_STEP(5, T_) NS_STEP(6, T_) NS_STEP(7, T_)
     }
-#define NS_TAIL(U) if constexpr (U < R - 1) { if (rem > U) step(std::integral_constant<int, U>{}, F_{}); }
+#define NS_TAIL(U) if constexpr (U < R - 1) { if (rem > U) step(std::integral_constant<int, U>{}, F_{}, X0_{}); }
     NS_TAIL(0) NS_TAIL(1) NS_TAIL(2) NS_TAIL(3) NS_TAIL(4) NS_TAIL(5) NS_TAIL(6)
+#undef NS_TAIL
+    }
 #undef NS_STEP
-#undef NS_TAIL
     if constexpr (BF) asm volatile("s_waitcnt lgkmcnt(0)" : "+v"(Aq[0][0]), "+v"(Aq[0][AK - 1]), "+v"(Aq[1][0]), "+v"(Aq[1][AK - 1]) :: "memory");
     else asm volatile("s_waitcnt lgkmcnt(0)" : "+v"(Aq[0][0]), "+v"(Aq[1][0]) :: "memory");
     NS_STAMP();
diff --git a/linna_amd/nn.py b/linna_amd/nn.py
--- a/linna_amd/nn.py
+++ b/linna_amd/nn.py
@@ -413,6 +413,14 @@
     return bool(n)
 
 
+def program_trim(model, rows=16):
+    buf = C.create_string_buffer(65536)
+    n = _lib.load().linna_program_trim(program_layers(model), len(model.ops), model.in_size, int(rows), buf, len(buf))
+    if n < 0:
+        _lib.check(n)
+    return n, buf.value.decode()
+
+
 def describe_grad_bf16_program(model, rows=16):
     arr = program_layers(model)
     buf = C.create_string_buffer(8192)
```

Measured after the change: 77.72 million evals/s, median of 6. 1.02x the previous value.
